# Cardinal-Cryptography/zk-apps

Measured on AMD Instinct MI355X. Metric: shielder_withdraw_groth16_proofs_per_sec_2^20_constraints, higher is better.
Workload: dtype int: signed 28-bit limbs in 32-bit words, 64-bit column accumulators (Fr 255-bit / Fq 381-bit Montgomery); 1 GPU; single withdraw-shaped Groth16 proof, N=2^20 (7 Fr NTTs, 4 G1 MSM + 1 G2 MSM of 2^20-1 terms), 1 proof per step per GPU; relation=update_note (withdraw) with Poseidon-5 hashing, chain-padded to N, curve=BLS12-381, independent_proofs_per_rank=171, distinct_witnesses_per_rank=64, fresh_r_s_per_proof=True, proofs_in_flight_per_gpu=3, msm_schedule=A | B1 (over r*z) + L + H reduced together | B2 (G2)

## Files before the change

### zk-apps_amd/csrc/groth16.hip

```cpp
#include <stdlib.h>
#include <string.h>
#include <new>
#include <string>
#include <memory>
#include <chrono>
#include <functional>
#include <thread>
#include <vector>
#include "ctx.hpp"
#include "tune.hpp"
#include "host_pool.hpp"
#include "pairing.hpp"
#include "r1cs.hpp"
#include "points.hpp"

namespace zkmi {

template <class T>
__device__ __forceinline__ T ldv(const T* p) {
  T r;
  const uint4* s = reinterpret_cast<const uint4*>(p);
  uint4* d = reinterpret_cast<uint4*>(&r);
#pragma unroll
  for (unsigned i = 0; i < sizeof(T) / 16; i++) d[i] = s[i];
  return r;
}
template <class T>
__device__ __forceinline__ void stv(T* p, const T& v) {
  const uint4* s = reinterpret_cast<const uint4*>(&v);
  uint4* d = reinterpret_cast<uint4*>(p);
#pragma unroll
  for (unsigned i = 0; i < sizeof(T) / 16; i++) d[i] = s[i];
}

struct MatSet {
  const uint32_t* rowptr[3];
  const uint32_t* col[3];
  const Fr28* val[3];
};
constexpr uint32_t MATVEC_LONG_ROW = 1024;
__global__ void __launch_bounds__(256)
k_matvec_long(MatSet ms, const uint32_t* __restrict__ rows, const Fr28* __restrict__ z, Fr28* __restrict__ out_base, uint32_t n, uint32_t n_vars) {
  __shared__ Fr28 part[256];
  const uint32_t m = rows[2 * blockIdx.x], i = rows[2 * blockIdx.x + 1];
  const uint32_t* __restrict__ col = ms.col[m];
  const Fr28* __restrict__ val = ms.val[m];
  z += (size_t)blockIdx.y * n_vars;
  Fr28 acc = Fr28::zero();
  const uint32_t b = ms.rowptr[m][i], e = ms.rowptr[m][i + 1];
  for (uint32_t k = b + threadIdx.x; k < e; k += 256) acc = acc + ld28(val + k) * ld28(z + col[k]);
  part[threadIdx.x] = acc;
  __syncthreads();
  for (int o = 128; o > 0; o >>= 1) {
    if ((int)threadIdx.x < o) part[threadIdx.x] = part[threadIdx.x] + part[threadIdx.x + o];
    __syncthreads();
  }
  if (threadIdx.x == 0) st28(out_base + (size_t)m * gridDim.y * n + (size_t)blockIdx.y * n + i, part[0]);
}

template <int S>
__global__ void __launch_bounds__(256)
k_matvec(MatSet ms, const Fr28* __restrict__ z, Fr28* __restrict__ out_base, uint32_t nc, uint32_t n, uint32_t n_pub,
         uint32_t n_vars) {
  const int m = blockIdx.z;
  const uint32_t* __restrict__ rowptr = ms.rowptr[m];
  const uint32_t* __restrict__ col = ms.col[m];
  const Fr28* __restrict__ val = ms.val[m];
  const int is_a = m == 0;
  Fr28* __restrict__ out = out_base + (size_t)m * gridDim.y * n;
  z += (size_t)blockIdx.y * n_vars;
  out += (size_t)blockIdx.y * n;
  const uint32_t gi = blockIdx.x * blockDim.x + threadIdx.x;
  const uint32_t i = gi / S, lane = gi % S;
  if (i >= n) return;
  Fr28 acc = Fr28::zero();
  if (i < nc) {
    const uint32_t b = rowptr[i], e = rowptr[i + 1];
    if (e - b > MATVEC_LONG_ROW) return;
    for (uint32_t k = b + lane; k < e; k += S) acc = acc + ld28(val + k) * ld28(z + col[k]);
  } else if (is_a && i < nc + n_pub && lane == 0) {
    acc = ld28(z + (i - nc));
  }
  if constexpr (S > 1) {
#pragma unroll
    for (int o = S / 2; o > 0; o >>= 1) {
      Fr28 t;
#pragma unroll
      for (int q = 0; q < Fr28::NL; q++) t.l[q] = __shfl_xor(acc.l[q], o);
      acc = acc + t;
    }
    if (lane != 0) return;
  }
  st28(out + i, acc);
}

__global__ void __launch_bounds__(256)
k_check_sat(const Fr28* __restrict__ a, const Fr28* __restrict__ b, const Fr28* __restrict__ c,
            const Fr28* __restrict__ z, uint32_t nc, uint32_t* __restrict__ flag, uint32_t n, uint32_t n_vars) {
  a += (size_t)blockIdx.y * n;
  b += (size_t)blockIdx.y * n;
  c += (size_t)blockIdx.y * n;
  z += (size_t)blockIdx.y * n_vars;
  const uint32_t i = blockIdx.x * blockDim.x + threadIdx.x;
  bool bad = false;
  if (i < nc) {
    const Fr28 d = (ld28(a + i) * ld28(b + i) - ld28(c + i)) * Fr28::one();
    bad = !d.is_zero();
  }
  if (i == 0) {
    const Fr28 d = (ld28(z) - Fr28::one()) * Fr28::one();
    bad = bad || !d.is_zero();
  }
  if (bad) __hip_atomic_fetch_or(flag, 1u, __ATOMIC_RELAXED, __HIP_MEMORY_SCOPE_SYSTEM);
}

__global__ void __launch_bounds__(256)
k_check_canonical(const uint32_t* __restrict__ z, uint32_t n, uint32_t* __restrict__ flag) {
  const uint32_t i = blockIdx.x * blockDim.x + threadIdx.x;
  if (i >= n) return;
  const uint4* q = reinterpret_cast<const uint4*>(z + (size_t)i * 8);
  const uint4 a = q[0], b = q[1];
  const uint32_t w[8] = {a.x, a.y, a.z, a.w, b.x, b.y, b.z, b.w};
  bool lt = false, decided = false;
#pragma unroll
  for (int k = 7; k >= 0; k--)
    if (!decided && w[k] != Fr28Params::MOD32[k]) {
      lt = w[k] < Fr28Params::MOD32[k];
      decided = true;
    }
  if (!lt) __hip_atomic_fetch_or(flag, 2u, __ATOMIC_RELAXED, __HIP_MEMORY_SCOPE_SYSTEM);
}

__global__ void __launch_bounds__(256)
k_quotient(Fr28* __restrict__ a, const Fr28* __restrict__ b, const Fr28* __restrict__ c, Fr28 zinv, uint32_t n) {
  const uint32_t i = blockIdx.x * blockDim.x + threadIdx.x;
  if (i >= n) return;
  st28(a + i, (ld28(a + i) * ld28(b + i) - ld28(c + i)) * zinv);
}

struct ZPtrSet {
  const uint4* p[64];
};
__global__ void __launch_bounds__(64)
k_gather_z(ZPtrSet src, uint4* __restrict__ dst, uint32_t vec16) {
  const uint32_t i = blockIdx.x * 64 + threadIdx.x;
  if (i >= vec16) return;
  dst[(size_t)blockIdx.y * vec16 + i] = src.p[blockIdx.y][i];
}

struct RSet {
  Fr28 r[64];
};
__global__ void __launch_bounds__(64)
k_scale_canonical(const uint32_t* __restrict__ in, RSet rs, uint32_t* __restrict__ out, uint32_t n, uint64_t stride) {
  const uint32_t i = blockIdx.x * 64 + threadIdx.x;
  if (i >= n) return;
  const size_t at = (size_t)blockIdx.y * stride + (size_t)i * 8;
  const uint4* q = reinterpret_cast<const uint4*>(in + at);
  const uint4 a = q[0], b = q[1];
  const uint32_t w[8] = {a.x, a.y, a.z, a.w, b.x, b.y, b.z, b.w};
  const Fr28 v = Fr28::from_canonical(w) * rs.r[blockIdx.y];
  uint32_t o[8];
  v.to_canonical(o);
  uint4* d = reinterpret_cast<uint4*>(out + at);
  d[0] = make_uint4(o[0], o[1], o[2], o[3]);
  d[1] = make_uint4(o[4], o[5], o[6], o[7]);
}

__global__ void __launch_bounds__(64)
k_entries_to_host(const uint32_t* __restrict__ part_total, uint32_t np, uint32_t* __restrict__ host_word) {
  uint32_t s = 0;
  for (uint32_t i = threadIdx.x; i < np; i += 64) s += part_total[i];
  for (int o = 32; o; o >>= 1) s += __shfl_down(s, o, 64);
  if (threadIdx.x == 0) __hip_atomic_store(host_word, s, __ATOMIC_RELAXED, __HIP_MEMORY_SCOPE_SYSTEM);
}

template <class A>
__global__ void __launch_bounds__(256)
k_bitrev_points(const A* __restrict__ in, A* __restrict__ out, int log_n) {
  const uint32_t p = blockIdx.x * blockDim.x + threadIdx.x;
  if (p >= (1u << log_n)) return;
  const uint32_t r = log_n ? (__brev(p) >> (32 - log_n)) : 0u;
  stv(out + p, ldv(in + r));
}

template <class F>
__global__ void __launch_bounds__(64)
k_fixed_base(const uint32_t* __restrict__ scalars, const Affine<F>* __restrict__ table, Affine<F>* __restrict__ out,
             uint32_t n) {
  const uint32_t i = blockIdx.x * blockDim.x + threadIdx.x;
  if (i >= n) return;
  XYZZ<F> acc = XYZZ<F>::infinity();
  for (int w = 0; w < 32; w++) {
    const uint32_t limb = scalars[(size_t)i * 8 + (w >> 2)];
    const uint32_t d = (limb >> ((w & 3) * 8)) & 0xffu;
    if (d) {
      Affine<F> p = ldv(table + w * 256 + d);
      acc.madd(p);
    }
  }
  stv(out + i, acc.to_affine());
}

}

using namespace zkmi;

static bool prover_sort_side() { return ZK_TUNE("ZKMI_SORT_SIDE", 0) == 1; }
static uint32_t prover_solo_max_log() {
  const int v = ZK_TUNE("ZKMI_SOLO_MAX_LOG", 19);
  return (uint32_t)(v < 0 ? 0 : v > 28 ? 28 : v);
}
static bool prover_aux_split() { return ZK_TUNE("ZKMI_AUX_SPLIT", 1) != 0; }

static bool same_bucket_set(const MsmPlan& a, const MsmPlan& b) {
  return a.shared == b.shared && a.c == b.c && a.nwin == b.nwin && a.nb == b.nb && a.seg_log == b.seg_log &&
         a.vec_parts == b.vec_parts && a.ndigits == b.ndigits;
}

struct zkmi_pk {
  zkmi_ctx* ctx = nullptr;
  int device = -1;
  uint32_t n_vars = 0, n_pub = 0, nc = 0, log_n = 0;
  uint32_t tree_height = 0;
  uint32_t gmax = 1;
  uint32_t* d_rowptr[3] = {nullptr, nullptr, nullptr};
  uint32_t* d_long_rows = nullptr;
  uint32_t n_long_rows = 0;
  uint32_t* d_col[3] = {nullptr, nullptr, nullptr};
  Fr28* d_val[3] = {nullptr, nullptr, nullptr};
  G1Affine *a_query = nullptr, *b_g1_query = nullptr, *h_query = nullptr, *l_query = nullptr;
  G2Affine* b_g2_query = nullptr;
  Affine<Fq28>*a28 = nullptr, *b1_28 = nullptr, *h28 = nullptr, *h28_rev = nullptr, *l28 = nullptr;
  Affine<Fq2_28>* b2_28 = nullptr;
  bool shared = false;
  Affine<Fq28>*a_tab = nullptr, *b1_tab = nullptr, *l_tab = nullptr, *h_tab = nullptr;
  Affine<Fq2_28>* b2_tab = nullptr;
  G1Affine alpha_g1, beta_g1, delta_g1, a0, b1_0;
  G2Affine beta_g2, delta_g2, b2_0;
  std::unique_ptr<FixedBase8<Fq>> delta1_tab, k1_tab;
  std::unique_ptr<FixedBase8<Fq2>> delta2_tab;
  G1Affine ka;
  G2Affine kb2;
  Fr* d_z[zkmi_ctx::PROOF_RING] = {};
  mutable const Fr* z_cur[zkmi_ctx::PROOF_RING] = {};
  uint32_t* d_rz[zkmi_ctx::PROOF_RING] = {};
  uint32_t* d_h[zkmi_ctx::PROOF_RING] = {};
  Fr28 *d_zm = nullptr, *d_a = nullptr;
  uint32_t* h_unsat = nullptr;
  uint32_t* h_zent = nullptr;
  mutable bool fold_dense = true;
  mutable uint64_t last_entries = 0, last_full = 0;
  ~zkmi_pk() {
    if (device >= 0) (void)hipSetDevice(device);
    (void)hipDeviceSynchronize();
    for (int m = 0; m < 3; m++) {
      if (d_rowptr[m]) (void)hipFree(d_rowptr[m]);
      if (d_col[m]) (void)hipFree(d_col[m]);
      if (d_val[m]) (void)hipFree(d_val[m]);
    }
    if (d_long_rows) (void)hipFree(d_long_rows);
    void* ptrs[] = {a_query, b_g1_query, h_query, l_query, b_g2_query, d_zm, d_a, a28, b1_28, h28, h28_rev, l28, b2_28,
                    a_tab, b1_tab, l_tab, h_tab, b2_tab, d_z[0], d_z[1], d_z[2], d_h[0], d_h[1], d_h[2]};
    static_assert(zkmi_ctx::PROOF_RING == 3, "ring size");
    for (void* p : ptrs)
      if (p) (void)hipFree(p);
    if (h_unsat) (void)hipHostFree(h_unsat);
    for (uint32_t* p : d_rz)
      if (p) (void)hipFree(p);
  }
};

static hipError_t pk_alloc(zkmi_pk* pk, zkmi_ctx* ctx, const zkmi_r1cs* r) {
  pk->ctx = ctx;
  pk->device = ctx->device;
  pk->n_vars = r->n_vars;
  pk->n_pub = r->n_pub;
  pk->nc = r->n_constraints;
  pk->log_n = r->log_n;
  pk->tree_height = r->tree_height;
  const uint64_t N = 1ull << r->log_n;
  hipError_t e;
  {
    std::vector<uint32_t> longs;
    for (uint32_t m = 0; m < 3; m++)
      for (uint32_t i = 0; i + 1 < r->m[m].rowptr.size(); i++)
        if (r->m[m].rowptr[i + 1] - r->m[m].rowptr[i] > MATVEC_LONG_ROW) {
          longs.push_back(m);
          longs.push_back(i);
        }
// ... 384 lines not shown
  }
  pk_build_delta_tables(pk);
  *out_pk = pk;
  return ZKMI_OK;
}

extern "C" {

int32_t zkmi_pk_check(zkmi_ctx* ctx, const zkmi_pk* pk, int32_t checks, uint64_t out_where[2]) {
  if (!ctx || !pk || checks == 0 || !point_args_ok(PT_ENC_RESIDENT, &checks)) return ZKMI_ERR_BAD_ARG;
  ZK_ENTER(ctx);
  if (ctx->device != pk->device) return ZKMI_ERR_BAD_ARG;
  if (out_where) out_where[0] = out_where[1] = UINT64_MAX;
  const bool sub = (checks & ZKMI_CHECK_SUBGROUP) != 0;
  const G1Affine* s1[3] = {&pk->alpha_g1, &pk->beta_g1, &pk->delta_g1};
  const G2Affine* s2[2] = {&pk->beta_g2, &pk->delta_g2};
  for (uint64_t i = 0; i < 5; i++) {
    const bool curve = i < 3 ? g1_on_curve(*s1[i]) : g2_on_curve(*s2[i - 3]);
    const bool ok = curve && (!sub || (i < 3 ? g1_in_subgroup(*s1[i]) : g2_in_subgroup(*s2[i - 3])));
    if (!ok) {
      if (out_where) out_where[0] = 5, out_where[1] = i;
      return ctx->fail(ZKMI_ERR_NON_CANONICAL, "proving key: single element " + std::to_string(i) + " (section 5): " +
                                                   point_status_name(curve ? ZKMI_PT_NOT_IN_SUBGROUP : ZKMI_PT_NOT_ON_CURVE));
    }
  }
  const uint64_t N = 1ull << pk->log_n, nv = pk->n_vars, np = pk->n_pub;
  struct {
    int group;
    const void* src;
    uint64_t cnt;
  } const sec[5] = {{1, pk->a_query, nv}, {1, pk->b_g1_query, nv}, {2, pk->b_g2_query, nv}, {1, pk->h_query, N - 1},
                    {1, pk->l_query + np, nv - np}};
  for (int k = 0; k < 5; k++) {
    if (!sec[k].cnt) continue;
    uint64_t bad = UINT64_MAX;
    uint32_t st = 0;
    const int32_t rc = points_read(ctx, sec[k].group, sec[k].src, sec[k].cnt, PT_ENC_RESIDENT, checks, nullptr, false, nullptr, &bad, &st);
    if (rc != ZKMI_OK) return rc;
    if (bad != UINT64_MAX) {
      if (out_where) out_where[0] = (uint64_t)k, out_where[1] = bad;
      return ctx->fail(ZKMI_ERR_NON_CANONICAL, std::string("proving key: ") + PK_QUERY_NAME[k] + "[" + std::to_string(bad) +
                                                   "] (section " + std::to_string(k) + "): " + point_status_name(st));
    }
  }
  return ZKMI_OK;
}

int32_t zkmi_pk_free(zkmi_pk* pk) {
  if (!pk) return ZKMI_ERR_BAD_ARG;
  delete pk;
  return ZKMI_OK;
}

int32_t zkmi_pk_shape(const zkmi_pk* pk, uint32_t* n_vars, uint32_t* n_pub, uint32_t* log_n) {
  if (!pk) return ZKMI_ERR_BAD_ARG;
  if (n_vars) *n_vars = pk->n_vars;
  if (n_pub) *n_pub = pk->n_pub;
  if (log_n) *log_n = pk->log_n;
  return ZKMI_OK;
}

int32_t zkmi_pk_schedule_state(const zkmi_pk* pk, uint64_t out[3]) {
  if (!pk || !out) return ZKMI_ERR_BAD_ARG;
  out[0] = (pk->d_rz[0] != nullptr && pk->fold_dense) ? 1 : 0;
  out[1] = pk->last_entries;
  out[2] = pk->last_full;
  return ZKMI_OK;
}

int32_t zkmi_ctx_set_group_size(zkmi_ctx* ctx, uint32_t group) {
  if (!ctx || group > 64) return ZKMI_ERR_BAD_ARG;
  ctx->group_override = group;
  return ZKMI_OK;
}

int32_t zkmi_pk_export_g1_elems(const zkmi_pk* pk, uint8_t out_beta_g1[96], uint8_t out_delta_g1[96]) {
  if (!pk || !out_beta_g1 || !out_delta_g1) return ZKMI_ERR_BAD_ARG;
  g1_to_wire(pk->beta_g1, out_beta_g1);
  g1_to_wire(pk->delta_g1, out_delta_g1);
  return ZKMI_OK;
}

int32_t zkmi_pk_export_query(zkmi_ctx* ctx, const zkmi_pk* pk, int32_t which, uint64_t first, uint64_t count,
                             uint8_t* out) {
  ZK_ENTER(ctx);
  if (!ctx || !pk || !out || which < 0 || which > 4) return ZKMI_ERR_BAD_ARG;
  const uint64_t N = 1ull << pk->log_n;
  if (which == 2) {
    if (first + count > pk->n_vars) return ZKMI_ERR_BAD_ARG;
    std::vector<G2Affine> h(count);
    ZK_HIP(ctx, hipMemcpy(h.data(), pk->b_g2_query + first, sizeof(G2Affine) * count, hipMemcpyDeviceToHost));
    for (uint64_t i = 0; i < count; i++) g2_to_wire(h[i], out + 192 * i);
    return ZKMI_OK;
  }
  const G1Affine* src = which == 0 ? pk->a_query : which == 1 ? pk->b_g1_query : which == 3 ? pk->h_query : pk->l_query + pk->n_pub;
  const uint64_t len = which == 3 ? N - 1 : which == 4 ? pk->n_vars - pk->n_pub : pk->n_vars;
  if (first + count > len) return ZKMI_ERR_BAD_ARG;
  std::vector<G1Affine> h(count);
  ZK_HIP(ctx, hipMemcpy(h.data(), src + first, sizeof(G1Affine) * count, hipMemcpyDeviceToHost));
  for (uint64_t i = 0; i < count; i++) g1_to_wire(h[i], out + 96 * i);
  return ZKMI_OK;
}

static int32_t witness_map_dev(zkmi_ctx* ctx, const zkmi_pk* pk, const void* const* src, bool host, uint32_t G,
                               hipStream_t st, int par = 0) {
  const uint32_t N = 1u << pk->log_n, nv = pk->n_vars;
  PhaseTimer* t = ctx->timer();
  pk->z_cur[par] = pk->d_z[par];
  bool aligned = true;
  for (uint32_t b = 0; b < G; b++) aligned = aligned && (reinterpret_cast<uintptr_t>(src[b]) & 15u) == 0;
  if (host) {
    for (uint32_t b = 0; b < G; b++)
      ZK_HIP(ctx, hipMemcpyAsync(pk->d_z[par] + (size_t)b * nv, src[b], 32ull * nv, hipMemcpyHostToDevice, ctx->stream_copy));
  } else if (G == 1 && aligned) {
    pk->z_cur[par] = static_cast<const Fr*>(src[0]);
  } else if (G <= 64 && aligned) {
    ZPtrSet ps;
    for (uint32_t b = 0; b < 64; b++) ps.p[b] = static_cast<const uint4*>(src[b < G ? b : 0]);
    hipLaunchKernelGGL(k_gather_z, dim3((2 * nv + 63) / 64, G), dim3(64), 0, ctx->stream_copy, ps, reinterpret_cast<uint4*>(pk->d_z[par]), 2 * nv);
  } else {
    for (uint32_t b = 0; b < G; b++)
      ZK_HIP(ctx, hipMemcpyAsync(pk->d_z[par] + (size_t)b * nv, src[b], 32ull * nv, hipMemcpyDeviceToDevice, ctx->stream_copy));
  }
  ZK_HIP(ctx, hipEventRecord(ctx->ev_z[par], ctx->stream_copy));
  ZK_HIP(ctx, hipStreamWaitEvent(ctx->stream, ctx->ev_z[par], 0));
  if (st != ctx->stream) ZK_HIP(ctx, hipStreamWaitEvent(st, ctx->ev_z[par], 0));
  if (t) t->begin(PH_WITNESS, st);
  hipLaunchKernelGGL(k_check_canonical, dim3((G * nv + 63) / 64), dim3(64), 0, st,
                     reinterpret_cast<const uint32_t*>(pk->z_cur[par]), G * nv, pk->h_unsat + par);
  ZK_HIP(ctx, ntt_from_canonical(reinterpret_cast<const uint32_t*>(pk->z_cur[par]), pk->d_zm, G * nv, st));
  MatSet ms;
  for (int m = 0; m < 3; m++) {
    ms.rowptr[m] = pk->d_rowptr[m];
    ms.col[m] = pk->d_col[m];
    ms.val[m] = pk->d_val[m];
  }
  if (G == 1 && pk->log_n <= 16)
    hipLaunchKernelGGL(k_matvec<8>, dim3((8 * N + 63) / 64, 1, 3), dim3(64), 0, st, ms, pk->d_zm, pk->d_a, pk->nc, N, pk->n_pub, nv);
  else
    hipLaunchKernelGGL(k_matvec<1>, dim3((N + 63) / 64, G, 3), dim3(64), 0, st, ms, pk->d_zm, pk->d_a, pk->nc, N, pk->n_pub, nv);
  if (pk->n_long_rows) hipLaunchKernelGGL(k_matvec_long, dim3(pk->n_long_rows, G), dim3(256), 0, st, ms, pk->d_long_rows, pk->d_zm, pk->d_a, N, nv);
  Fr28* const d_b = pk->d_a + (size_t)N * G;
  Fr28* const d_c = pk->d_a + 2 * (size_t)N * G;
  hipLaunchKernelGGL(k_check_sat, dim3((pk->nc + 64) / 64, G), dim3(64), 0, st, pk->d_a, d_b, d_c, pk->d_zm, pk->nc,
                     pk->h_unsat + par, N, nv);
  if (t) t->end(PH_WITNESS, st);
  hipError_t e;
  NttDomain* dom = ctx->domain((int)pk->log_n, &e);
  if (!dom) return ctx->hip_fail(e, "ntt domain");
  if (t) t->begin(PH_NTT, st);
  const bool batch_abc = ZK_TUNE("ZKMI_WITNESS_BATCH", 1) != 0;
  if (batch_abc) {
    ZK_HIP(ctx, dom->inverse_to_rev(pk->d_a, dom->rev_coset_n, nullptr, st, 3 * G));
    ZK_HIP(ctx, dom->forward_from_rev(pk->d_a, st, 3 * G));
  } else {
    for (int m = 0; m < 3; m++) {
      ZK_HIP(ctx, dom->inverse_to_rev(pk->d_a + (size_t)m * N * G, dom->rev_coset_n, nullptr, st, G));
      ZK_HIP(ctx, dom->forward_from_rev(pk->d_a + (size_t)m * N * G, st, G));
    }
  }
  Fr gn = fr_from_u64(7);
  for (uint32_t i = 0; i < pk->log_n; i++) gn = gn.sqr();
  const Fr zinv = (gn - Fr::one()).inv().from_mont();
  const Fr28 zinv28 = Fr28::from_canonical(zinv.l);
  hipLaunchKernelGGL(k_quotient, dim3((G * N + 63) / 64), dim3(64), 0, st, pk->d_a, d_b, d_c, zinv28, G * N);
  ZK_HIP(ctx, dom->inverse_to_rev(pk->d_a, dom->rev_coset_inv_n, pk->d_h[par], st, G));
  if (t) t->end(PH_NTT, st);
  if (st != ctx->stream) ZK_HIP(ctx, hipEventRecord(ctx->ev_h[par], st));
  ZK_HIP(ctx, hipGetLastError());
  return ZKMI_OK;
}

int32_t zkmi_groth16_witness_map(zkmi_ctx* ctx, const zkmi_pk* pk, const uint8_t* z, uint8_t* out_h) {
  ZK_ENTER(ctx);
  if (!ctx || !pk || !z || !out_h) return ZKMI_ERR_BAD_ARG;
  const void* src[1] = {z};
  int32_t rc = witness_map_dev(ctx, pk, src, true, 1, ctx->stream);
  if (rc != ZKMI_OK) return rc;
  const uint32_t N = 1u << pk->log_n;
  std::vector<uint8_t> rev(32ull * N);
  ZK_HIP(ctx, hipMemcpyAsync(rev.data(), pk->d_h[0], 32ull * N, hipMemcpyDeviceToHost, ctx->stream));
  ZK_HIP(ctx, hipStreamSynchronize(ctx->stream));
  const uint32_t flags0 = pk->h_unsat[0];
  pk->h_unsat[0] = 0;
  if (flags0 & 2u) return ctx->fail(ZKMI_ERR_NON_CANONICAL, "witness element >= r");
  for (uint32_t p = 0; p < N; p++) {
    uint32_t i = 0;
    for (uint32_t b = 0; b < pk->log_n; b++) i |= ((p >> b) & 1u) << (pk->log_n - 1 - b);
    memcpy(out_h + 32ull * i, rev.data() + 32ull * p, 32);
  }
  return ZKMI_OK;
}

static int32_t prove_enqueue_z(zkmi_ctx* ctx, const zkmi_pk* pk, const void* const* src, bool host, uint32_t G, int par, bool solo = false,
                               bool followed = false, const uint8_t* r_bytes = nullptr) {
  const uint32_t nv = pk->n_vars;
  hipStream_t st = ctx->stream;
  int32_t rc = witness_map_dev(ctx, pk, src, host, G, ctx->stream_front, par);
  if (rc != ZKMI_OK) return rc;
  PhaseTimer* t = ctx->timer();
  const int s0 = 4 * par, g2s = par;
  const bool heavy_side = ZK_TUNE("ZKMI_HEAVY_ON", 2) == 1;
  if (heavy_side) ZK_HIP(ctx, ctx->lazy_stream(&ctx->stream_heavy, false));
  const hipStream_t sth = heavy_side ? ctx->stream_heavy : nullptr;
  const uint32_t* zs = reinterpret_cast<const uint32_t*>(pk->z_cur[par] + 1);
  const bool sh = pk->shared;
  const bool sort_side = prover_sort_side();
  MsmSort& sz = (sort_side && (ctx->z_flip++ & 1u)) ? ctx->sort_z2 : ctx->sort;
  const bool aux_split = prover_aux_split();
  const hipStream_t ra = ctx->stream_aux, rb = aux_split ? ctx->stream_aux2 : ctx->stream_aux,
                    rc2 = aux_split ? ctx->stream_aux3 : ctx->stream_aux;
  if (sort_side) ZK_HIP(ctx, ctx->lazy_stream(&ctx->stream_sort, true));
  const hipStream_t ss = sort_side ? ctx->stream_sort : st;
  if (sort_side) ZK_HIP(ctx, hipStreamWaitEvent(ss, ctx->ev_z[par], 0));
  if (G > 1)
    ZK_HIP(ctx, sz.run_shared_batch(zs, nv - 1, 8ull * nv, G, ss, t));
  else if (sh)
    ZK_HIP(ctx, sz.run_shared(zs, nv - 1, ss, t));
  else
    ZK_HIP(ctx, sz.run(zs, nv - 1, ss, t));
  if (sh && pk->d_rz[par]) hipLaunchKernelGGL(k_entries_to_host, dim3(1), dim3(64), 0, ss, sz.part_total, (uint32_t)sz.plan.nwin, pk->h_zent + par);
  ZK_HIP(ctx, hipEventRecord(ctx->ev_sort[par], ss));
  if (sort_side) ZK_HIP(ctx, hipStreamWaitEvent(st, ctx->ev_sort[par], 0));
  ZK_HIP(ctx, hipStreamWaitEvent(ctx->stream_g2, ctx->ev_sort[par], 0));
  const bool spread_on = ZK_TUNE("ZKMI_SPREAD", 1) != 0;
  const bool spread = spread_on && G == 1 && pk->log_n <= (solo ? prover_solo_max_log() : 16u) && !sort_side && sh;
  const bool three_streams = spread && !solo;
  if (three_streams) ZK_HIP(ctx, ctx->lazy_stream(&ctx->stream_acc3, false));
  const hipStream_t sb1 = three_streams ? ctx->stream_copy : st, sl = three_streams ? ctx->stream_acc3 : st;
  if (three_streams) {
    ZK_HIP(ctx, hipStreamWaitEvent(sb1, ctx->ev_sort[par], 0));
    ZK_HIP(ctx, hipStreamWaitEvent(sl, ctx->ev_sort[par], 0));
  }
  if (spread && solo) {
    ZK_HIP(ctx, ctx->sort_h.run_shared(pk->d_h[par], 1u << pk->log_n, ctx->stream_front, t));
    ZK_HIP(ctx, hipEventRecord(ctx->ev_sorth[par], ctx->stream_front));
    const bool g2_early = ZK_TUNE("ZKMI_SOLO_G2_EARLY", 1) != 0;
    if (!g2_early) ZK_HIP(ctx, hipStreamWaitEvent(ctx->stream_g2, ctx->ev_sorth[par], 0));
    ZK_HIP(ctx, hipStreamWaitEvent(st, ctx->ev_sorth[par], 0));
    ZK_HIP(ctx, ctx->g2.run_device(sz, pk->b2_tab, ctx->stream_g2, rc2, t, PH_MSM_ACCUM_G2, PH_MSM_REDUCE_G2, g2s, sth));
    const MsmPlan &pz = sz.plan, &ph = ctx->sort_h.plan;
    const bool fuse_h = ZK_TUNE("ZKMI_SOLO_FUSE_H", 1) != 0;
    const bool fused = fuse_h && same_bucket_set(pz, ph);
    ctx->h_mode[par] = fused ? zkmi_ctx::H_FUSED : zkmi_ctx::H_SORTED;
    const MsmSort* sorts[4] = {&sz, &sz, &sz, &ctx->sort_h};
    const Affine<Fq28>* tabs[4] = {pk->a_tab, pk->b1_tab, pk->l_tab, pk->h_tab};
    const hipStream_t reds[4] = {ra, rb, ctx->stream_front, ctx->stream_copy};
    const int slots4[4] = {s0 + 0, s0 + 1, s0 + 2, s0 + 3};
    ZK_HIP(ctx, ctx->g1.run_device_multi(sorts, tabs, fused ? 4 : 3, st, reds, t, PH_MSM_ACCUM_G1, PH_MSM_REDUCE_G1, slots4, sth));
    return ZKMI_OK;
  }
  const int lh_mode = ZK_TUNE("ZKMI_LH_MERGE", 2);
  const uint32_t N = 1u << pk->log_n;
  const bool same_set = sh && same_bucket_set(sz.plan, G > 1 ? msm_make_plan_shared_batch(N, G) : msm_make_plan_shared(N));
  const bool nocall_g1 = ZK_TUNE("ZKMI_ACCUM", 3) == 2 || ZK_TUNE("ZKMI_ACCUM", 3) == 3;
  const bool lh_merge = same_set && ((lh_mode == 2 && !solo) ||
                                     (lh_mode == 1 && nocall_g1 && followed && (G == 1 || ZK_TUNE("ZKMI_LH_MERGE_GROUPS", 0) == 1)));
  const bool fold_b1 = lh_merge && lh_mode == 2 && r_bytes && pk->d_rz[par] != nullptr && (pk->fold_dense || ZK_TUNE("ZKMI_RB1_FOLD_ALWAYS", 0) == 1);
  ctx->h_mode[par] = fold_b1 ? zkmi_ctx::H_INTO_LB : lh_merge ? zkmi_ctx::H_INTO_L : zkmi_ctx::H_OWN;
  if (fold_b1) {
    RSet rs;
    for (uint32_t g = 0; g < G; g++) {
      uint32_t rw[8];
      memcpy(rw, r_bytes + 32ull * g, 32);
      rs.r[g] = Fr28::from_canonical(rw);
    }
    const bool own = ZK_TUNE("ZKMI_RB1_STREAM", 0) == 1;
    if (own) {
      ZK_HIP(ctx, ctx->lazy_stream(&ctx->stream_rz, false));
      ZK_HIP(ctx, hipStreamWaitEvent(ctx->stream_rz, ctx->ev_z[par], 0));
    }
    const hipStream_t sc = own ? ctx->stream_rz : ctx->stream_copy;
    hipLaunchKernelGGL(k_scale_canonical, dim3((nv - 1 + 63) / 64, G), dim3(64), 0, sc, zs, rs, pk->d_rz[par], nv - 1, 8ull * nv);
    if (G > 1)
      ZK_HIP(ctx, ctx->sort_rz.run_shared_batch(pk->d_rz[par], nv - 1, 8ull * nv, G, sc, t));
    else
      ZK_HIP(ctx, ctx->sort_rz.run_shared(pk->d_rz[par], nv - 1, sc, t));
    ZK_HIP(ctx, hipEventRecord(ctx->ev_rz[par], sc));
  }
  ZK_HIP(ctx, ctx->g2.run_device(sz, sh ? pk->b2_tab : pk->b2_28 + 1, ctx->stream_g2, rc2, t,
                                 PH_MSM_ACCUM_G2, PH_MSM_REDUCE_G2, g2s, sth));
  ZK_HIP(ctx, ctx->g1.run_device(sz, sh ? pk->a_tab : pk->a28 + 1, st, ra, t, PH_MSM_ACCUM_G1,
                                 PH_MSM_REDUCE_G1, s0 + 0, sth));
  if (fold_b1) {
    ZK_HIP(ctx, hipStreamWaitEvent(sb1, ctx->ev_rz[par], 0));
    ZK_HIP(ctx, ctx->g1.run_device(ctx->sort_rz, pk->b1_tab, sb1, rb, t, PH_MSM_ACCUM_G1, PH_MSM_REDUCE_G1, s0 + 1, sth, -1, MSM_RUN_NO_REDUCE));
  } else {
    ZK_HIP(ctx, ctx->g1.run_device(sz, sh ? pk->b1_tab : pk->b1_28 + 1, sb1, lh_merge ? ra : rb, t, PH_MSM_ACCUM_G1,
                                   PH_MSM_REDUCE_G1, s0 + 1, sth));
  }
  ZK_HIP(ctx, ctx->g1.run_device(sz, sh ? pk->l_tab : pk->l28 + 1, sl, lh_merge ? rb : ra, t, PH_MSM_ACCUM_G1,
                                 PH_MSM_REDUCE_G1, s0 + 2, sth, -1, lh_merge ? MSM_RUN_NO_REDUCE : 0));
  return ZKMI_OK;
}

static int32_t prove_enqueue_h(zkmi_ctx* ctx, const zkmi_pk* pk, uint32_t G, int par, bool solo = false) {
  const uint32_t N = 1u << pk->log_n;
  (void)solo;
  const int mode = ctx->h_mode[par];
  if (mode == zkmi_ctx::H_FUSED) return ZKMI_OK;
  const bool spread = mode == zkmi_ctx::H_SORTED;
  hipStream_t st = spread ? ctx->stream_copy : ctx->stream;
  if (spread) ZK_HIP(ctx, hipStreamWaitEvent(st, ctx->ev_sorth[par], 0));
  PhaseTimer* t = ctx->timer();
  const bool sh = pk->shared;
  const bool heavy_side = ZK_TUNE("ZKMI_HEAVY_ON", 2) == 1;
  if (heavy_side) ZK_HIP(ctx, ctx->lazy_stream(&ctx->stream_heavy, false));
  const hipStream_t sth = heavy_side ? ctx->stream_heavy : nullptr;
  const bool sort_side = prover_sort_side();
  if (sort_side) ZK_HIP(ctx, ctx->lazy_stream(&ctx->stream_sort, true));
  const hipStream_t ss = sort_side ? ctx->stream_sort : st;
  ZK_HIP(ctx, hipStreamWaitEvent(ss, ctx->ev_h[par], 0));
  if (spread)
    ;
  else if (G > 1)
    ZK_HIP(ctx, ctx->sort_h.run_shared_batch(pk->d_h[par], N, 8ull * N, G, ss, t));
  else if (sh)
    ZK_HIP(ctx, ctx->sort_h.run_shared(pk->d_h[par], N, ss, t));
  else
// ... 503 lines not shown
```

### zk-apps_amd/csrc/msm.hpp

```cpp
#pragma once
#include <hip/hip_runtime.h>
#include <stdint.h>
#include <vector>
#include "curve.hpp"
#include "field28.hpp"
#include "tune.hpp"

namespace zkmi {

struct PhaseTimer {
  enum { MAX_PENDING = 4096 };
  hipEvent_t ev0[MAX_PENDING], ev1[MAX_PENDING];
  int phase_of[MAX_PENDING];
  int n_pending = 0, n_created = 0;
  bool enabled = false;
  double total_ms[16] = {0};
  uint64_t count[16] = {0};
  ~PhaseTimer();
  void begin(int phase, hipStream_t st);
  void end(int phase, hipStream_t st);
  void collect();
  void reset();
};

enum Phase {
  PH_MSM_SORT = 0,
  PH_MSM_ACCUM_G1 = 1,
  PH_MSM_REDUCE_G1 = 2,
  PH_MSM_ACCUM_G2 = 3,
  PH_MSM_REDUCE_G2 = 4,
  PH_NTT = 5,
  PH_WITNESS = 6,
  PH_MISC = 7,
  PH_COUNT = 8
};

constexpr uint64_t MSM_MAX_TERMS = (1ull << 28) - 1;

constexpr int MSM_BIG_WINDOW = 20;
constexpr int MSM_MAX_WINDOW = 22;

struct MsmPlan {
  int c = 0;
  int nwin = 0;
  uint32_t nb = 0;
  uint64_t n = 0;
  bool shared = false;
  int ndigits = 0;
  uint32_t heavy_thr = 256;
  int heavy_shift = 0;
  int seg_log = 4;
  int vec_parts = 1;
  int top_spread_log = 0;
  int win_first = 0, nwin_total = 0;
  int total_windows() const { return nwin_total ? nwin_total : nwin; }
};
MsmPlan msm_make_plan(uint64_t n);
MsmPlan msm_make_plan_c(uint64_t n, int c);
MsmPlan msm_make_plan_shared(uint64_t n);
MsmPlan msm_make_plan_shared_batch(uint64_t n, uint32_t batch);

struct MsmSort {
  uint32_t* count = nullptr;
  uint32_t* begin = nullptr;
  uint32_t* blockhist = nullptr;
  uint32_t* perm = nullptr;
  uint32_t* heavy = nullptr;
  uint32_t* order_bins = nullptr;
  uint32_t* part_total = nullptr;
  uint32_t* blkcnt = nullptr;
  uint32_t* fpart = nullptr;
  uint32_t* rec_entry = nullptr;
  uint32_t* rec_bkt = nullptr;
  uint32_t* rec_aux = nullptr;
  uint32_t* big_ws = nullptr;
  uint32_t* sorted = nullptr;
  uint64_t cap_entries = 0, cap_buckets = 0, cap_hist = 0;
  MsmPlan plan;
  int plan_override = 0;
  int win_first = 0, win_count = 0;
  int big_nb_log = 15;
  mutable std::vector<hipEvent_t> readers;
  hipError_t wait_readers(hipStream_t st);
  ~MsmSort() { release(); }
  void release();
  bool has_shared = false;
  hipError_t reserve(uint64_t n, bool shared_too = false);
  hipError_t allocate(uint64_t ne, uint64_t nbk, uint64_t nh, bool shared);
  hipError_t run(const uint32_t* d_scalars, uint64_t n, hipStream_t st, PhaseTimer* prof);
  hipError_t run_windowed_big(const uint32_t* d_scalars, uint64_t n, hipStream_t st, PhaseTimer* prof);
  hipError_t run_shared(const uint32_t* d_scalars, uint64_t n, hipStream_t st, PhaseTimer* prof);
  hipError_t run_shared_batch(const uint32_t* d_scalars, uint64_t n, uint64_t stride_words, uint32_t batch, hipStream_t st,
                              PhaseTimer* prof);
  hipError_t reserve_batch(uint64_t n, uint32_t batch);
};

hipError_t msm_sort_enable_big_lds();

template <class F> struct HostFieldOf;
template <> struct HostFieldOf<Fq28> { using type = Fq; };
template <> struct HostFieldOf<Fq2_28> { using type = Fq2; };
template <> struct HostFieldOf<BnFq28> { using type = BnFq; };

enum { MSM_RUN_NO_REDUCE = 1, MSM_RUN_ADD_AT_REDUCE = 2, MSM_RUN_TWO_WAVES = 4 };

template <class F>
struct MsmEngine {
  using HF = typename HostFieldOf<F>::type;
  enum { SLOTS = 12, SLOT_PTS = 64 * 32 };
  int nslots = SLOTS;
  XYZZ<F>* buckets = nullptr;
  XYZZ<F>* segsum = nullptr;
  XYZZ<F>* segw = nullptr;
  uint64_t seg_cap = 0;
  XYZZ<F>* heavy_partial = nullptr;
  uint32_t* heavy_ticket = nullptr;
  uint32_t* heavy_plan = nullptr;
  XYZZ<HF>* partial = nullptr;
  XYZZ<F>* tree_stage = nullptr;
  XYZZ<HF>* h_partial = nullptr;
  hipEvent_t done[SLOTS] = {};
  hipEvent_t acc_done[SLOTS] = {};
  hipEvent_t pre[SLOTS] = {};
  hipEvent_t heavy_done[SLOTS] = {};
  hipEvent_t redo_done[SLOTS] = {};
  uint32_t* redo = nullptr;
  MsmPlan slot_plan[SLOTS];
  bool host_spin = true;
  uint64_t cap_buckets = 0;
  uint64_t min_buckets = 0;
  ~MsmEngine() {
    release();
    destroy_events();
  }
  void release();
  hipError_t reset_transients();
  void destroy_events();
  bool has_shared = false;
  hipError_t reserve(uint64_t n, bool shared_too = false);
  hipError_t reserve_buckets(uint64_t buckets);
  hipError_t ensure_slots(int n);
  hipError_t run_device(const MsmSort& sort, const Affine<F>* d_bases, hipStream_t st, hipStream_t st_reduce,
                        PhaseTimer* prof, int ph_accum, int ph_reduce, int slot = 0, hipStream_t st_heavy = nullptr,
                        int bucket_slot = -1, int flags = 0, int bucket_slot3 = -1);
  hipError_t run_device_multi(const MsmSort* const* sorts, const Affine<F>* const* d_bases, int nm, hipStream_t st,
                              const hipStream_t* st_reduces, PhaseTimer* prof, int ph_accum, int ph_reduce, const int* slots,
                              hipStream_t st_heavy = nullptr, const int* bucket_slots = nullptr, int flags = 0, int third_slot = -1);
  hipError_t finish_host(XYZZ<HF>* out, int slot = 0);
  hipError_t finish_host_windows(XYZZ<HF>* out_windows, int slot = 0);
  static void windows_from_partials(const MsmPlan& pl, const XYZZ<HF>* h, XYZZ<HF>* out_windows, bool parallel = false);
  static int partials_per_msm(const MsmPlan& pl);
  hipError_t finish_host_batch(XYZZ<HF>* out, int slot = 0);
  hipError_t wait_slot(int slot);
  XYZZ<HF> host_result_vec(int slot, int v) const;
};

template <class F>
hipError_t bases_convert(const Affine<typename HostFieldOf<F>::type>* d_in, Affine<F>* d_out, uint64_t n, hipStream_t st);

template <class HF>
XYZZ<HF> msm_combine_windows(const XYZZ<HF>* windows, int nwin, int c);

template <class F>
hipError_t msm_build_table(const Affine<F>* d_bases, uint64_t n, const MsmPlan& plan, Affine<F>** out_table,
                           hipStream_t st);

extern template struct MsmEngine<Fq28>;
extern template struct MsmEngine<Fq2_28>;
extern template struct MsmEngine<BnFq28>;
extern template hipError_t msm_build_table<Fq28>(const Affine<Fq28>*, uint64_t, const MsmPlan&, Affine<Fq28>**, hipStream_t);
extern template hipError_t msm_build_table<Fq2_28>(const Affine<Fq2_28>*, uint64_t, const MsmPlan&, Affine<Fq2_28>**, hipStream_t);
extern template hipError_t msm_build_table<BnFq28>(const Affine<BnFq28>*, uint64_t, const MsmPlan&, Affine<BnFq28>**, hipStream_t);
extern template hipError_t bases_convert<Fq28>(const Affine<Fq>*, Affine<Fq28>*, uint64_t, hipStream_t);
extern template hipError_t bases_convert<Fq2_28>(const Affine<Fq2>*, Affine<Fq2_28>*, uint64_t, hipStream_t);
extern template hipError_t bases_convert<BnFq28>(const Affine<BnFq>*, Affine<BnFq28>*, uint64_t, hipStream_t);

}
```

### zk-apps_amd/csrc/msm_impl.hpp

```cpp
#pragma once
#include <stdlib.h>
#include <functional>
#include <type_traits>
#include <vector>
#include "curve.hpp"
#include "host_pool.hpp"
#include "msm.hpp"

namespace zkmi {

static inline uint64_t msm_max_segments(uint64_t buckets) { return (buckets / 16 > (1u << 16) ? buckets / 16 : (1u << 16)) + 1; }
constexpr int MSM_TREE_T = 128;
constexpr uint32_t MSM_STAGE_PTS = 16384;
constexpr uint32_t MSM_STAGE_PTS_1 = 4096;
constexpr uint32_t MSM_HEAVY = 256;

template <class T>
__device__ __forceinline__ T load_vec(const T* p) {
  static_assert(sizeof(T) % 16 == 0, "16-byte multiple");
  T r;
  const uint4* s = reinterpret_cast<const uint4*>(p);
  uint4* d = reinterpret_cast<uint4*>(&r);
#pragma unroll
  for (unsigned i = 0; i < sizeof(T) / 16; i++) d[i] = s[i];
  return r;
}
template <class T>
__device__ __forceinline__ void store_vec(T* p, const T& v) {
  static_assert(sizeof(T) % 16 == 0, "16-byte multiple");
  const uint4* s = reinterpret_cast<const uint4*>(&v);
  uint4* d = reinterpret_cast<uint4*>(p);
#pragma unroll
  for (unsigned i = 0; i < sizeof(T) / 16; i++) d[i] = s[i];
}

typedef __attribute__((address_space(3))) void* lds_ptr_t;
typedef const __attribute__((address_space(1))) void* glb_ptr_t;


__device__ __forceinline__ Fq28 ld_comp(const Fq28* p) {
  Fq28 r;
  const uint2* q = reinterpret_cast<const uint2*>(p);
#pragma unroll
  for (int i = 0; i < 7; i++) {
    const uint2 w = q[i];
    r.l[2 * i] = (int32_t)w.x;
    r.l[2 * i + 1] = (int32_t)w.y;
  }
  return r;
}
__device__ __forceinline__ void st_comp(Fq28* p, const Fq28& v) {
  uint2* q = reinterpret_cast<uint2*>(p);
#pragma unroll
  for (int i = 0; i < 7; i++) q[i] = make_uint2((uint32_t)v.l[2 * i], (uint32_t)v.l[2 * i + 1]);
}


template <class F>
__device__ __forceinline__ bool madd_generic(XYZZ<F>& acc, const Affine<F>& p, uint32_t negmask = 0) {
  F pp_ = f_sub_lazy(p.x * acc.zz, acc.x);
  F r = f_signed_sub_lazy(p.y * acc.zzz, negmask, acc.y);
  F pp = pp_.sqr();
  F rr = r.sqr();
  if (pp.is_zero()) return false;
  F ppp = pp_ * pp;
  acc.zz = acc.zz * pp;
  acc.zzz = acc.zzz * ppp;
  F q = acc.x * pp;
  acc.x = f_x3(rr, ppp, q);
  acc.y = f_mul_sub_mul(r, f_sub_lazy(q, acc.x), acc.y, ppp);
  return true;
}
template <class F>
__device__ __forceinline__ bool madd_affine_pair(XYZZ<F>& acc, const Affine<F>& p, uint32_t negmask = 0) {
  F pp_ = f_sub_lazy(p.x, acc.x);
  F r = f_signed_sub_lazy(p.y, negmask, acc.y);
  F pp = pp_.sqr();
  F rr = r.sqr();
  if (pp.is_zero()) return false;
  F ppp = pp_ * pp;
  F q = acc.x * pp;
  acc.x = f_x3(rr, ppp, q);
  acc.y = f_mul_sub_mul(r, f_sub_lazy(q, acc.x), acc.y, ppp);
  acc.zz = pp;
  acc.zzz = ppp;
  return true;
}
template <class P>
__device__ __forceinline__ bool affine_is_zero_words(const Affine<Fp28<P>>& p) {
  if (p.y.l[0] != 0) return false;
  uint32_t o = 0;
#pragma unroll
  for (int i = 0; i < P::NL; i++) o |= (uint32_t)p.x.l[i] | (uint32_t)p.y.l[i];
  return o == 0;
}

constexpr int MSM_MULTI_MAX = 4;
struct SortView {
  const uint32_t *begin, *count, *perm, *sorted;
  uint32_t heavy_thr;
};
template <class F, bool MULTI>
struct AccumArgs;
template <class F>
struct AccumArgs<F, false> {
  const Affine<F>* bases_;
  XYZZ<F>* buckets_;
  uint32_t* redo_;
  SortView sort_;
  __device__ __forceinline__ const Affine<F>* bases() const { return bases_; }
  __device__ __forceinline__ XYZZ<F>* buckets() const { return buckets_; }
  __device__ __forceinline__ uint32_t* redo() const { return redo_; }
  __device__ __forceinline__ const SortView& sort() const { return sort_; }
};
template <class F>
struct AccumArgs<F, true> {
  const Affine<F>* bases_[MSM_MULTI_MAX];
  XYZZ<F>* buckets_[MSM_MULTI_MAX];
  uint32_t* redo_[MSM_MULTI_MAX];
  SortView sort_[MSM_MULTI_MAX];
  __device__ __forceinline__ const Affine<F>* bases() const { return bases_[blockIdx.y]; }
  __device__ __forceinline__ XYZZ<F>* buckets() const { return buckets_[blockIdx.y]; }
  __device__ __forceinline__ uint32_t* redo() const { return redo_[blockIdx.y]; }
  __device__ __forceinline__ const SortView& sort() const { return sort_[blockIdx.y]; }
};
template <class F, int W, int BW, bool MULTI = false, bool INTO = false>
__global__ void __launch_bounds__(64 * BW, W)
k_accum_g1_nc(const AccumArgs<F, MULTI> args, uint32_t total_buckets) {
  const Affine<F>* __restrict__ const bases = args.bases();
  XYZZ<F>* __restrict__ const buckets = args.buckets();
  uint32_t* __restrict__ const redo = args.redo();
  const uint32_t* __restrict__ const begin = args.sort().begin;
  const uint32_t* __restrict__ const count = args.sort().count;
  const uint32_t* __restrict__ const perm = args.sort().perm;
  const uint32_t* __restrict__ const sorted = args.sort().sorted;
  const uint32_t heavy_thr = args.sort().heavy_thr;
  constexpr int CHUNKS = sizeof(Affine<F>) / 16;
  __shared__ uint4 tile[BW][CHUNKS][64];
  const uint32_t t = blockIdx.x * blockDim.x + threadIdx.x;
  const uint32_t wave = threadIdx.x >> 6, lane = threadIdx.x & 63;
  if (t >= total_buckets) return;
  const uint32_t b = perm[t];
  const uint32_t cnt = count[b];
  if (cnt > heavy_thr) return;
  const uint32_t beg = begin[b], end = beg + cnt;
  auto fetch = [&](uint32_t v) {
    const char* src = reinterpret_cast<const char*>(bases + (v & 0x7fffffffu));
#pragma unroll
    for (int q = 0; q < CHUNKS; q++)
      __builtin_amdgcn_global_load_lds((glb_ptr_t)(src + 16 * q), (lds_ptr_t)&tile[wave][q][0], 16, 0, 0);
  };
  auto take = [&](Affine<F>& p) {
    uint4* d = reinterpret_cast<uint4*>(&p);
#pragma unroll
    for (int q = 0; q < CHUNKS; q++) d[q] = tile[wave][q][lane];
    asm volatile("s_waitcnt lgkmcnt(0)" ::: "memory");
  };
  XYZZ<F> acc;
  uint32_t j = beg;
  for (;; j++) {
    if (j >= end) {
      if constexpr (!INTO) store_vec(buckets + b, XYZZ<F>::infinity());
      return;
    }
// ... 672 lines not shown
        if (sv >> 31) p.y = p.y.neg();
        v.madd(p);
      }
    }
    return v;
  };
  const uint32_t n_heavy = pmode ? hplan[2] : (heavy[0] < h_limit ? heavy[0] : h_limit);
  auto put = [&](uint32_t b, XYZZ<F> v) {
    if (into) v.add(load_vec(buckets + b));
    store_vec(buckets + b, v);
  };
  const uint32_t n_wg = gridDim.x * gridDim.y, wg = blockIdx.y * gridDim.x + blockIdx.x;
  uint32_t item0 = 0;
  const bool tail = h_first >= MSM_HEAVY_CAP;
  for (uint32_t h = tail ? h_first + wg : h_first; h < n_heavy; h += tail ? n_wg : 1u) {
    const uint32_t b = pmode ? ent[4 * h] : heavy[1 + h];
    const uint32_t cnt = pmode ? (ent[4 * (h + 1) + 3] - ent[4 * h + 3]) * 64u : count[b];
    const uint32_t beg0 = pmode ? ent[4 * h + 3] * 64u : begin[b];
    const uint32_t nsplit = tail ? 1u : heavy_nsplit(h, cnt, 4 * MSM_TREE_T, item0);
    const uint32_t base = item0;
    const uint32_t r0 = tail ? 0u : (wg + n_wg - base % n_wg) % n_wg;
    item0 += nsplit;
    for (uint32_t r = r0; r < nsplit; r += n_wg) {
      uint32_t beg = beg0, end = beg0 + cnt;
      if (nsplit > 1) {
        const uint32_t len = (cnt + nsplit - 1) / nsplit;
        const uint32_t sb = beg + r * len;
        end = (sb + len < end) ? sb + len : end;
        beg = sb < end ? sb : end;
      }
      XYZZ<F> acc = XYZZ<F>::infinity();
      if (pmode) {
        for (uint32_t j = beg + threadIdx.x; j < end; j += blockDim.x) acc.add(partial_at(h, j));
      } else {
        for (uint32_t j = beg + threadIdx.x; j < end; j += blockDim.x) {
          const uint32_t v = sorted[j];
          Affine<F> p = load_vec(bases + (v & 0x7fffffffu));
          if (v >> 31) p.y = p.y.neg();
          acc.madd(p);
        }
      }
      acc = block_tree_sum(acc, sh);
      if (nsplit == 1) {
        if (threadIdx.x == 0) put(b, acc);
      } else {
        if (threadIdx.x == 0) {
          store_vec(heavy_partial + (size_t)base + r, acc);
          __threadfence();
          is_last = atomicAdd(ticket + h, 1u) == nsplit - 1 ? 1u : 0u;
        }
        __syncthreads();
        if (is_last) {
          __threadfence();
          XYZZ<F> v = XYZZ<F>::infinity();
          for (uint32_t k = threadIdx.x; k < nsplit; k += blockDim.x) v.add(load_vec(heavy_partial + (size_t)base + k));
          v = block_tree_sum(v, sh);
          if (threadIdx.x == 0) {
            put(b, v);
            ticket[h] = 0;
          }
        }
      }
      __syncthreads();
    }
  }
}

template <class F>
__global__ void __launch_bounds__(256)
k_segreduce(const XYZZ<F>* __restrict__ buckets, XYZZ<F>* __restrict__ segsum, XYZZ<F>* __restrict__ segw,
            uint32_t total_segs, int seg, const XYZZ<F>* __restrict__ buckets2, const XYZZ<F>* __restrict__ buckets3) {
  const uint32_t t = blockIdx.x * blockDim.x + threadIdx.x;
  if (t >= total_segs) return;
  XYZZ<F> run = XYZZ<F>::infinity();
  XYZZ<F> acc = XYZZ<F>::infinity();
  for (int i = seg - 1; i >= 0; i--) {
    XYZZ<F> bk = load_vec(buckets + (size_t)t * seg + i);
    run.add(bk);
    if (buckets2) {
      bk = load_vec(buckets2 + (size_t)t * seg + i);
      run.add(bk);
    }
    if (buckets3) {
      bk = load_vec(buckets3 + (size_t)t * seg + i);
      run.add(bk);
    }
    acc.add(run);
  }
  store_vec(segsum + t, run);
  store_vec(segw + t, acc);
}

template <class F>
__global__ void __launch_bounds__(256, 2)
k_segreduce_w2(const XYZZ<F>* __restrict__ buckets, XYZZ<F>* __restrict__ segsum, XYZZ<F>* __restrict__ segw,
            uint32_t total_segs, int seg, const XYZZ<F>* __restrict__ buckets2, const XYZZ<F>* __restrict__ buckets3) {
  const uint32_t t = blockIdx.x * blockDim.x + threadIdx.x;
  if (t >= total_segs) return;
  XYZZ<F> run = XYZZ<F>::infinity();
  XYZZ<F> acc = XYZZ<F>::infinity();
  for (int i = seg - 1; i >= 0; i--) {
    XYZZ<F> bk = load_vec(buckets + (size_t)t * seg + i);
    run.add(bk);
    if (buckets2) {
      bk = load_vec(buckets2 + (size_t)t * seg + i);
      run.add(bk);
    }
    if (buckets3) {
      bk = load_vec(buckets3 + (size_t)t * seg + i);
      run.add(bk);
    }
    acc.add(run);
  }
  store_vec(segsum + t, run);
  store_vec(segw + t, acc);
}

__device__ __forceinline__ XYZZ<Fq2P> ld_xyzz_split(const XYZZ<Fq2_28>* p, uint32_t comp) {
  const Fq28* s = reinterpret_cast<const Fq28*>(p);
  XYZZ<Fq2P> r;
  r.x.v = ld_comp(s + comp);
  r.y.v = ld_comp(s + 2 + comp);
  r.zz.v = ld_comp(s + 4 + comp);
  r.zzz.v = ld_comp(s + 6 + comp);
  return r;
}
__device__ __forceinline__ void st_xyzz_split(XYZZ<Fq2_28>* p, const XYZZ<Fq2P>& v, uint32_t comp) {
  Fq28* d = reinterpret_cast<Fq28*>(p);
  st_comp(d + comp, v.x.v);
  st_comp(d + 2 + comp, v.y.v);
  st_comp(d + 4 + comp, v.zz.v);
  st_comp(d + 6 + comp, v.zzz.v);
}

template <int UNUSED = 0>
__global__ void __launch_bounds__(256, 2)
k_segreduce_g2_split(const XYZZ<Fq2_28>* __restrict__ buckets, XYZZ<Fq2_28>* __restrict__ segsum,
                     XYZZ<Fq2_28>* __restrict__ segw, uint32_t total_segs, int seg) {
  const uint32_t gt = blockIdx.x * blockDim.x + threadIdx.x;
  const uint32_t t = gt >> 1, comp = gt & 1u;
  if (t >= total_segs) return;
  XYZZ<Fq2P> run = XYZZ<Fq2P>::infinity();
  XYZZ<Fq2P> acc = XYZZ<Fq2P>::infinity();
  for (int i = seg - 1; i >= 0; i--) {
    XYZZ<Fq2P> bk = ld_xyzz_split(buckets + (size_t)t * seg + i, comp);
    run.add(bk);
    acc.add(run);
  }
  st_xyzz_split(segsum + t, run, comp);
  st_xyzz_split(segw + t, acc, comp);
}

template <class F>
__global__ void __launch_bounds__(MSM_TREE_T)
k_treesum(const XYZZ<F>* __restrict__ segsum, const XYZZ<F>* __restrict__ segw, uint32_t segs_per_win,
          XYZZ<typename HostFieldOf<F>::type>* __restrict__ partial, int plain_job, XYZZ<F>* __restrict__ stage,
          XYZZ<typename HostFieldOf<F>::type>* __restrict__ partial_host) {
  extern __shared__ __align__(16) unsigned char lds_raw[];
  XYZZ<F>* sh = reinterpret_cast<XYZZ<F>*>(lds_raw);
  const int job = blockIdx.x;
  const int w = blockIdx.y;
  const uint32_t nchunk = gridDim.z, z = blockIdx.z;
  const XYZZ<F>* src = (job == 0 ? segw : segsum) + (size_t)w * segs_per_win;
  const bool whole = job == 0 || job == plain_job;
  const uint32_t len = whole ? segs_per_win : segs_per_win / 2;
  const uint32_t per = (len + nchunk - 1) / nchunk;
  const uint32_t lo = z * per, hi = lo + per < len ? lo + per : len;
  XYZZ<F> acc = XYZZ<F>::infinity();
  if (whole) {
    for (uint32_t t = lo + threadIdx.x; t < hi; t += blockDim.x) {
      XYZZ<F> v = load_vec(src + t);
      acc.add(v);
    }
  } else {
    const uint32_t b = (uint32_t)(job - 1), lowmask = (1u << b) - 1u;
    for (uint32_t u = lo + threadIdx.x; u < hi; u += blockDim.x) {
      const uint32_t t = ((u & ~lowmask) << 1) | (1u << b) | (u & lowmask);
      XYZZ<F> v = load_vec(src + t);
      acc.add(v);
    }
  }
  sh[threadIdx.x] = acc;
  __syncthreads();
  for (uint32_t s = blockDim.x / 2; s > 0; s >>= 1) {
    if (threadIdx.x < s) {
      acc.add(sh[threadIdx.x + s]);
      sh[threadIdx.x] = acc;
    }
    __syncthreads();
  }
  if (threadIdx.x == 0) {
    if (nchunk == 1) {
      XYZZ<typename HostFieldOf<F>::type> o = {fq_from_fq28(acc.x), fq_from_fq28(acc.y), fq_from_fq28(acc.zz),
                                               fq_from_fq28(acc.zzz)};
      store_vec(partial + (size_t)w * gridDim.x + job, o);
      store_vec(partial_host + (size_t)w * gridDim.x + job, o);
    } else {
      store_vec(stage + ((size_t)w * gridDim.x + job) * nchunk + z, acc);
    }
  }
}

template <class F>
__global__ void __launch_bounds__(MSM_TREE_T)
k_treesum_final(const XYZZ<F>* __restrict__ stage, uint32_t nchunk, XYZZ<typename HostFieldOf<F>::type>* __restrict__ partial,
                XYZZ<typename HostFieldOf<F>::type>* __restrict__ partial_host) {
  extern __shared__ __align__(16) unsigned char lds_raw[];
  XYZZ<F>* sh = reinterpret_cast<XYZZ<F>*>(lds_raw);
  const size_t idx = (size_t)blockIdx.y * gridDim.x + blockIdx.x;
  XYZZ<F> acc = XYZZ<F>::infinity();
  if (threadIdx.x < nchunk) acc = load_vec(stage + idx * nchunk + threadIdx.x);
  sh[threadIdx.x] = acc;
  __syncthreads();
  for (uint32_t s = blockDim.x / 2; s > 0; s >>= 1) {
    if (threadIdx.x < s) {
      acc.add(sh[threadIdx.x + s]);
      sh[threadIdx.x] = acc;
    }
    __syncthreads();
  }
  if (threadIdx.x == 0) {
    XYZZ<typename HostFieldOf<F>::type> o = {fq_from_fq28(acc.x), fq_from_fq28(acc.y), fq_from_fq28(acc.zz),
                                             fq_from_fq28(acc.zzz)};
    store_vec(partial + idx, o);
    store_vec(partial_host + idx, o);
  }
}

__device__ __forceinline__ void st_host_split(XYZZ<Fq2>* dst, const XYZZ<Fq2P>& v, uint32_t comp) {
  Fq* d = reinterpret_cast<Fq*>(dst);
  d[comp] = fq_from_fq28(v.x.v);
  d[2 + comp] = fq_from_fq28(v.y.v);
  d[4 + comp] = fq_from_fq28(v.zz.v);
  d[6 + comp] = fq_from_fq28(v.zzz.v);
}
__device__ __forceinline__ XYZZ<Fq2P> pair_tree_sum(XYZZ<Fq2P> acc, XYZZ<Fq2_28>* sh, uint32_t pair, uint32_t npair, uint32_t comp) {
  st_xyzz_split(sh + pair, acc, comp);
  __syncthreads();
  for (uint32_t s = npair / 2; s > 0; s >>= 1) {
    if (pair < s) {
      XYZZ<Fq2P> o = ld_xyzz_split(sh + pair + s, comp);
      acc.add(o);
      st_xyzz_split(sh + pair, acc, comp);
    }
    __syncthreads();
  }
  return acc;
}
template <int UNUSED = 0>
__global__ void __launch_bounds__(2 * MSM_TREE_T, 2)
k_treesum_g2_split(const XYZZ<Fq2_28>* __restrict__ segsum, const XYZZ<Fq2_28>* __restrict__ segw, uint32_t segs_per_win,
                   XYZZ<Fq2>* __restrict__ partial, int plain_job, XYZZ<Fq2_28>* __restrict__ stage, XYZZ<Fq2>* __restrict__ partial_host) {
  extern __shared__ __align__(16) unsigned char lds_raw[];
  XYZZ<Fq2_28>* sh = reinterpret_cast<XYZZ<Fq2_28>*>(lds_raw);
  const int job = blockIdx.x;
  const int w = blockIdx.y;
  const uint32_t nchunk = gridDim.z, z = blockIdx.z;
  const uint32_t pair = threadIdx.x >> 1, comp = threadIdx.x & 1u, npair = blockDim.x >> 1;
  const XYZZ<Fq2_28>* src = (job == 0 ? segw : segsum) + (size_t)w * segs_per_win;
  const bool whole = job == 0 || job == plain_job;
  const uint32_t len = whole ? segs_per_win : segs_per_win / 2;
  const uint32_t per = (len + nchunk - 1) / nchunk;
  const uint32_t lo = z * per, hi = lo + per < len ? lo + per : len;
  const uint32_t b = whole ? 0u : (uint32_t)(job - 1), lowmask = (1u << b) - 1u;
  XYZZ<Fq2P> acc = XYZZ<Fq2P>::infinity();
  for (uint32_t u = lo + pair; u < hi; u += npair) {
    const uint32_t t = whole ? u : (((u & ~lowmask) << 1) | (1u << b) | (u & lowmask));
    XYZZ<Fq2P> v = ld_xyzz_split(src + t, comp);
    acc.add(v);
  }
  acc = pair_tree_sum(acc, sh, pair, npair, comp);
  if (pair == 0) {
    if (nchunk == 1)
    {
      st_host_split(partial + (size_t)w * gridDim.x + job, acc, comp);
      st_host_split(partial_host + (size_t)w * gridDim.x + job, acc, comp);
    }
    else
      st_xyzz_split(stage + ((size_t)w * gridDim.x + job) * nchunk + z, acc, comp);
  }
}
template <int UNUSED = 0>
__global__ void __launch_bounds__(2 * MSM_TREE_T, 2)
k_treesum_final_g2_split(const XYZZ<Fq2_28>* __restrict__ stage, uint32_t nchunk, XYZZ<Fq2>* __restrict__ partial,
                         XYZZ<Fq2>* __restrict__ partial_host) {
  extern __shared__ __align__(16) unsigned char lds_raw[];
  XYZZ<Fq2_28>* sh = reinterpret_cast<XYZZ<Fq2_28>*>(lds_raw);
  const size_t idx = (size_t)blockIdx.y * gridDim.x + blockIdx.x;
  const uint32_t pair = threadIdx.x >> 1, comp = threadIdx.x & 1u, npair = blockDim.x >> 1;
  XYZZ<Fq2P> acc = XYZZ<Fq2P>::infinity();
  if (pair < nchunk) acc = ld_xyzz_split(stage + idx * nchunk + pair, comp);
  acc = pair_tree_sum(acc, sh, pair, npair, comp);
  if (pair == 0) {
    st_host_split(partial + idx, acc, comp);
    st_host_split(partial_host + idx, acc, comp);
  }
}

__device__ __forceinline__ Affine<Fq2P> ld_affine_split(const Affine<Fq2_28>* bases, uint32_t v, uint32_t comp) {
  const Fq28* src = reinterpret_cast<const Fq28*>(bases + (v & 0x7fffffffu));
  Affine<Fq2P> p;
  p.x.v = ld_comp(src + comp);
  p.y.v = ld_comp(src + 2 + comp);
  if (v >> 31) p.y = p.y.neg();
  return p;
}
template <int UNUSED = 0>
__global__ void __launch_bounds__(MSM_TREE_T, 2)
k_accum_heavy_g2_split(const Affine<Fq2_28>* __restrict__ bases, const uint32_t* __restrict__ begin,
                       const uint32_t* __restrict__ count, const uint32_t* __restrict__ heavy,
                       const uint32_t* __restrict__ sorted, XYZZ<Fq2_28>* __restrict__ buckets,
                       XYZZ<Fq2_28>* __restrict__ heavy_partial, uint32_t* __restrict__ ticket, uint32_t h_first,
                       uint32_t h_limit, const uint32_t* __restrict__ hplan, const XYZZ<Fq2_28>* __restrict__ pool_nc) {
  extern __shared__ __align__(16) unsigned char lds_raw[];
  XYZZ<Fq2_28>* sh = reinterpret_cast<XYZZ<Fq2_28>*>(lds_raw);
  __shared__ uint32_t is_last;
  const uint32_t pair = threadIdx.x >> 1, comp = threadIdx.x & 1u, npair = blockDim.x >> 1;
  const bool pmode = hplan != nullptr && hplan[3] == 0;
  const uint32_t* __restrict__ const ent = hplan + 4;
  const uint32_t pl_nc = pmode ? hplan[1] : 0u;
  auto partial_at = [&](uint32_t h, uint32_t j) {
    XYZZ<Fq2P> v = ld_xyzz_split(pool_nc + j, comp);
    uint32_t o = 0;
#pragma unroll
    for (int i = 0; i < Fq28::NL; i++) o |= (uint32_t)v.zz.v.l[i];
    uint32_t mk = (comp == 0 && v.zzz.v.l[0] == 1) ? 1u : 0u;
    o |= (uint32_t)__builtin_amdgcn_mov_dpp((int)o, 0xB1, 0xF, 0xF, true);
    mk |= (uint32_t)__builtin_amdgcn_mov_dpp((int)mk, 0xB1, 0xF, 0xF, true);
    if (o == 0 && mk == 1) {
      const uint32_t it = j >> 5, pr = j & 31u;
      const uint32_t beg = ent[4 * h + 1], cnt = ent[4 * h + 2], first = ent[4 * h + 3];
      const uint32_t w0 = beg + (it - first) * 32u * pl_nc;
      const uint32_t w1 = (w0 + 32u * pl_nc < beg + cnt) ? w0 + 32u * pl_nc : beg + cnt;
      v = XYZZ<Fq2P>::infinity();
      for (uint32_t jj = w0 + pr; jj < w1; jj += 32) v.madd(ld_affine_split(bases, sorted[jj], comp));
    } else if (o == 0) {
      v = XYZZ<Fq2P>::infinity();
    }
    return v;
  };
  const uint32_t n_heavy = pmode ? hplan[2] : (heavy[0] < h_limit ? heavy[0] : h_limit);
  const uint32_t n_wg = gridDim.x * gridDim.y, wg = blockIdx.y * gridDim.x + blockIdx.x;
  uint32_t item0 = 0;
  const bool tail = h_first >= MSM_HEAVY_CAP;
  for (uint32_t h = tail ? h_first + wg : h_first; h < n_heavy; h += tail ? n_wg : 1u) {
    const uint32_t b = pmode ? ent[4 * h] : heavy[1 + h];
    const uint32_t cnt = pmode ? (ent[4 * (h + 1) + 3] - ent[4 * h + 3]) * 32u : count[b];
    const uint32_t beg0 = pmode ? ent[4 * h + 3] * 32u : begin[b];
    const uint32_t nsplit = tail ? 1u : heavy_nsplit(h, cnt, 4 * npair, item0);
    const uint32_t base = item0;
    const uint32_t r0 = tail ? 0u : (wg + n_wg - base % n_wg) % n_wg;
    item0 += nsplit;
    for (uint32_t r = r0; r < nsplit; r += n_wg) {
      uint32_t beg = beg0, end = beg0 + cnt;
      if (nsplit > 1) {
        const uint32_t len = (cnt + nsplit - 1) / nsplit;
        const uint32_t sb = beg + r * len;
        end = (sb + len < end) ? sb + len : end;
        beg = sb < end ? sb : end;
      }
      XYZZ<Fq2P> acc = XYZZ<Fq2P>::infinity();
      if (pmode) {
        for (uint32_t j = beg + pair; j < end; j += npair) acc.add(partial_at(h, j));
      } else {
        for (uint32_t j = beg + pair; j < end; j += npair) acc.madd(ld_affine_split(bases, sorted[j], comp));
      }
      acc = pair_tree_sum(acc, sh, pair, npair, comp);
      if (nsplit == 1) {
        if (pair == 0) st_xyzz_split(buckets + b, acc, comp);
      } else {
        if (pair == 0) {
          st_xyzz_split(heavy_partial + (size_t)base + r, acc, comp);
          __threadfence();
        }
        __syncthreads();
        if (threadIdx.x == 0) is_last = atomicAdd(ticket + h, 1u) == nsplit - 1 ? 1u : 0u;
        __syncthreads();
        if (is_last) {
          __threadfence();
          XYZZ<Fq2P> v = XYZZ<Fq2P>::infinity();
          for (uint32_t k = pair; k < nsplit; k += npair) v.add(ld_xyzz_split(heavy_partial + (size_t)base + k, comp));
          v = pair_tree_sum(v, sh, pair, npair, comp);
          if (pair == 0) st_xyzz_split(buckets + b, v, comp);
          if (threadIdx.x == 0) ticket[h] = 0;
        }
      }
      __syncthreads();
    }
  }
}
template <int UNUSED = 0>
__global__ void __launch_bounds__(64, 2)
k_accum_redo_g2_split(const Affine<Fq2_28>* __restrict__ bases, const uint32_t* __restrict__ begin,
                      const uint32_t* __restrict__ count, const uint32_t* __restrict__ sorted,
                      XYZZ<Fq2_28>* __restrict__ buckets, uint32_t* __restrict__ redo, uint32_t* __restrict__ ticket) {
  extern __shared__ __align__(16) unsigned char lds_raw[];
  XYZZ<Fq2_28>* sh = reinterpret_cast<XYZZ<Fq2_28>*>(lds_raw);
  const uint32_t n = redo[0];
  const uint32_t pair = threadIdx.x >> 1, comp = threadIdx.x & 1u, npair = blockDim.x >> 1;
  for (uint32_t k = blockIdx.x; k < n; k += gridDim.x) {
    const uint32_t b = redo[1 + k];
    const uint32_t beg = begin[b], end = beg + count[b];
    XYZZ<Fq2P> acc = XYZZ<Fq2P>::infinity();
    for (uint32_t j = beg + pair; j < end; j += npair) acc.madd(ld_affine_split(bases, sorted[j], comp));
    acc = pair_tree_sum(acc, sh, pair, npair, comp);
    if (pair == 0) st_xyzz_split(buckets + b, acc, comp);
    __syncthreads();
  }
  __syncthreads();
  if (threadIdx.x == 0 && atomicAdd(ticket, 1u) == gridDim.x - 1) {
    redo[0] = 0;
    *ticket = 0;
  }
}

}
#include "msm_quad.hpp"
namespace zkmi {

template <class F>
__global__ void __launch_bounds__(256)
k_bases_convert(const Affine<typename HostFieldOf<F>::type>* __restrict__ in, Affine<F>* __restrict__ out,
                uint32_t n) {
  uint32_t i = blockIdx.x * blockDim.x + threadIdx.x;
  if (i >= n) return;
  Affine<typename HostFieldOf<F>::type> p = load_vec(in + i);
  Affine<F> q = {fq28_from_fq(p.x), fq28_from_fq(p.y)};
  store_vec(out + i, q);
}

template <class F>
void MsmEngine<F>::release() {
  if (buckets) (void)hipFree(buckets);
  if (segsum) (void)hipFree(segsum);
  if (segw) (void)hipFree(segw);
  if (partial) (void)hipFree(partial);
  if (tree_stage) (void)hipFree(tree_stage);
  tree_stage = nullptr;
  if (heavy_partial) (void)hipFree(heavy_partial);
  heavy_partial = nullptr;
  if (heavy_plan) (void)hipFree(heavy_plan);
  heavy_plan = nullptr;
  if (heavy_ticket) (void)hipFree(heavy_ticket);
  heavy_ticket = nullptr;
  if (redo) (void)hipFree(redo);
  redo = nullptr;
  if (h_partial) (void)hipHostFree(h_partial);
  buckets = segsum = segw = nullptr;
  partial = h_partial = nullptr;
  cap_buckets = 0;
}

uint64_t msm_max_buckets(uint64_t n);

template <class F>
hipError_t MsmEngine<F>::reset_transients() {
  if (!redo || !heavy_ticket) return hipSuccess;
  hipError_t e = hipMemset(redo, 0, sizeof(uint32_t) * (cap_buckets + 2) * nslots);
  if (e != hipSuccess) return e;
  return hipMemset(heavy_ticket, 0, sizeof(uint32_t) * MSM_HEAVY_CAP * nslots);
}

template <class F>
void MsmEngine<F>::destroy_events() {
  for (int i = 0; i < SLOTS; i++) {
    hipEvent_t* evs[] = {&done[i], &acc_done[i], &pre[i], &heavy_done[i], &redo_done[i]};
    for (hipEvent_t* e : evs) {
      if (*e) (void)hipEventDestroy(*e);
      *e = nullptr;
    }
  }
}

template <class F>
hipError_t MsmEngine<F>::ensure_slots(int n) {
  if (n > SLOTS) return hipErrorInvalidValue;
  if (n <= nslots) return hipSuccess;
  const bool sh = has_shared;
  const uint64_t mb = min_buckets;
  release();
  has_shared = sh;
  min_buckets = mb;
  nslots = n;
  return hipSuccess;
}

template <class F>
hipError_t MsmEngine<F>::reserve_buckets(uint64_t buckets) {
  if (buckets <= cap_buckets) return hipSuccess;
  const bool sh = has_shared;
  release();
  has_shared = sh;
  min_buckets = buckets;
  return reserve(1, sh);
}

template <class F>
hipError_t MsmEngine<F>::reserve(uint64_t n, bool shared_too) {
  uint64_t need = msm_max_buckets(n);
  if (need < min_buckets) need = min_buckets;
  const uint64_t forced = (uint64_t)(255 / 16 + 1) * (1u << 15);
  if (need < forced) need = forced;
  shared_too = shared_too || has_shared;
  if (shared_too) {
    const MsmPlan sp = msm_make_plan_shared(n);
    const uint64_t sb = (uint64_t)sp.nwin * sp.nb;
    if (need < sb) need = sb;
  }
  has_shared = shared_too;
  if (need <= cap_buckets) return hipSuccess;
  release();
  hipError_t e;
  if ((e = hipMalloc(&buckets, sizeof(XYZZ<F>) * need * nslots)) != hipSuccess) return e;
  seg_cap = msm_max_segments(need);
  if ((e = hipMalloc(&segsum, sizeof(XYZZ<F>) * seg_cap * nslots)) != hipSuccess) return e;
  if ((e = hipMalloc(&segw, sizeof(XYZZ<F>) * seg_cap * nslots)) != hipSuccess) return e;
  if ((e = hipMalloc(&partial, sizeof(XYZZ<HF>) * SLOTS * SLOT_PTS)) != hipSuccess) return e;
  if ((e = hipMalloc(&tree_stage, sizeof(XYZZ<F>) * MSM_STAGE_PTS * nslots)) != hipSuccess) return e;
  if ((e = hipMalloc(&heavy_partial, sizeof(XYZZ<F>) * ((size_t)MSM_HPOOL + MSM_HNC_POOL) * nslots)) != hipSuccess) return e;
  if ((e = hipMalloc(&heavy_plan, sizeof(uint32_t) * MSM_HPLAN_WORDS * nslots)) != hipSuccess) return e;
  if ((e = hipMalloc(&heavy_ticket, sizeof(uint32_t) * MSM_HEAVY_CAP * nslots)) != hipSuccess) return e;
  if ((e = hipMemset(heavy_ticket, 0, sizeof(uint32_t) * MSM_HEAVY_CAP * nslots)) != hipSuccess) return e;
  if ((e = hipMalloc(&redo, sizeof(uint32_t) * (need + 2) * nslots)) != hipSuccess) return e;
  if ((e = hipMemset(redo, 0, sizeof(uint32_t) * (need + 2) * nslots)) != hipSuccess) return e;
  if ((e = hipHostMalloc(&h_partial, sizeof(XYZZ<HF>) * SLOTS * SLOT_PTS, hipHostMallocCoherent)) != hipSuccess) return e;
  for (int i = 0; i < SLOTS; i++) {
    hipEvent_t* evs[] = {&done[i], &acc_done[i], &pre[i], &heavy_done[i], &redo_done[i]};
    for (hipEvent_t* ev : evs)
      if (!*ev && (e = hipEventCreateWithFlags(ev, hipEventDisableTiming)) != hipSuccess) return e;
  }
  cap_buckets = need;
  return hipSuccess;
}

static inline int msm_seg_bits(const MsmPlan& pl) {
  const uint32_t segs_per_win = pl.nb >> pl.seg_log;
  int seg_bits = 0;
  while ((1u << seg_bits) < segs_per_win) seg_bits++;
  return seg_bits;
}

template <class F>
hipError_t MsmEngine<F>::run_device(const MsmSort& sort, const Affine<F>* d_bases, hipStream_t st,
                                    hipStream_t st_reduce, PhaseTimer* prof, int ph_accum, int ph_reduce, int slot,
                                    hipStream_t st_heavy, int bucket_slot, int flags, int bucket_slot3) {
  const MsmSort* sp = &sort;
  return run_device_multi(&sp, &d_bases, 1, st, &st_reduce, prof, ph_accum, ph_reduce, &slot, st_heavy,
                          bucket_slot >= 0 ? &bucket_slot : nullptr, flags, bucket_slot3);
}

template <class F>
hipError_t MsmEngine<F>::run_device_multi(const MsmSort* const* sorts, const Affine<F>* const* d_bases, int nm, hipStream_t st,
                                          const hipStream_t* st_reduces, PhaseTimer* prof, int ph_accum, int ph_reduce,
                                          const int* slots, hipStream_t st_heavy, const int* bucket_slots, int flags, int third_slot) {
  if (nm < 1 || nm > MSM_MULTI_MAX) return hipErrorInvalidValue;
  if (third_slot >= nslots || (third_slot >= 0 && (nm != 1 || !(flags & MSM_RUN_ADD_AT_REDUCE) || !bucket_slots))) return hipErrorInvalidValue;
  const bool no_reduce = (flags & MSM_RUN_NO_REDUCE) != 0;
  const bool add_at_reduce = (flags & MSM_RUN_ADD_AT_REDUCE) != 0;
  bool any_into = false;
  for (int m = 0; m < nm; m++) {
    if (slots[m] < 0 || slots[m] >= nslots) return hipErrorInvalidValue;
    if (bucket_slots && (bucket_slots[m] < 0 || bucket_slots[m] >= nslots)) return hipErrorInvalidValue;
    any_into = any_into || (!add_at_reduce && bucket_slots && bucket_slots[m] != slots[m]);
  }
  if (add_at_reduce && std::is_same<F, Fq2_28>::value) return hipErrorInvalidValue;
  if (any_into && (nm != 1 || std::is_same<F, Fq2_28>::value)) return hipErrorInvalidValue;
  const MsmPlan& pl = sorts[0]->plan;
  for (int m = 1; m < nm; m++) {
    const MsmPlan& q = sorts[m]->plan;
    if (q.nwin != pl.nwin || q.nb != pl.nb || q.seg_log != pl.seg_log || q.shared != pl.shared || q.c != pl.c) return hipErrorInvalidValue;
  }
  const uint32_t tot_b = pl.nwin * pl.nb;
  const int T = 256;
  hipError_t e;
  const int heavy_on = ZK_TUNE("ZKMI_HEAVY_ON", 2);
  const int accum_mode = ZK_TUNE("ZKMI_ACCUM", 3);
  const int accum_mode_g2 = ZK_TUNE("ZKMI_ACCUM_G2", 2);
  const int mode = std::is_same<F, Fq2_28>::value ? accum_mode_g2 : accum_mode;
  const bool nocall = mode == 2 || mode == 3;
  constexpr bool g2_engine = std::is_same<F, Fq2_28>::value;
  const int quad_mask = g2_engine ? (host_spin ? ZK_TUNE("ZKMI_QUAD_G2", 15) : ZK_TUNE("ZKMI_QUAD_G2_BATCH", 12))
                                  : (host_spin ? ZK_TUNE("ZKMI_QUAD", 15) : ZK_TUNE("ZKMI_QUAD_BATCH", 12));
  using QPT = typename std::conditional<g2_engine, XYZZQ<Fq28, 0, true>, XYZZQ<F, 0, false>>::type;
  constexpr uint32_t QPW = g2_engine ? 8u : 16u;
  const bool quad_reduce_ok = pl.shared || pl.c <= 16;
#ifdef ZKMI_EXPERIMENTS
  const int accum_block = ZK_TUNE("ZKMI_ACCUM_BLOCK", 64) == 256 ? 256 : 64;
  const int accum_rounds = ZK_TUNE("ZKMI_ACCUM_ROUNDS", 0);
  auto striped = [&](uint32_t threads_needed, uint32_t block) {
    uint32_t blocks = (threads_needed + block - 1) / block;
    if (accum_rounds > 1) blocks = (blocks + accum_rounds - 1) / accum_rounds;
    return blocks ? blocks : 1u;
  };
#else
  if (!nocall) return hipErrorInvalidValue;
#endif
  if (any_into && !nocall) return hipErrorInvalidValue;
  auto bslot_of = [&](int m) { return bucket_slots ? bucket_slots[m] : slots[m]; };
  auto into_of = [&](int m) { return !add_at_reduce && bslot_of(m) != slots[m]; };
  auto second_of = [&](int m) { return add_at_reduce && bslot_of(m) != slots[m]; };
  auto bk_of = [&](int m) { return buckets + (size_t)(into_of(m) ? bslot_of(m) : slots[m]) * cap_buckets; };
  {
    const uint32_t spw = pl.nb >> pl.seg_log;
    if ((uint64_t)pl.nwin * spw > seg_cap || (uint64_t)(2 + msm_seg_bits(pl)) * pl.nwin > SLOT_PTS || tot_b > cap_buckets)
      return hipErrorInvalidValue;
  }
  auto redo_of = [&](int m) { return this->redo + (size_t)slots[m] * (cap_buckets + 2); };

  bool heavy_first[MSM_MULTI_MAX];
  hipStream_t heavy_stream[MSM_MULTI_MAX];
  const bool heavy_deferred = host_spin && tot_b <= (1u << 16) && (quad_mask & 8) && heavy_on == 2 && ZK_TUNE("ZKMI_HEAVY_DEFER", 0) != 0;
  auto launch_heavy = [&](int m) {
    const MsmSort& sort = *sorts[m];
    XYZZ<F>* const hp = heavy_partial + (size_t)slots[m] * ((size_t)MSM_HPOOL + MSM_HNC_POOL);
    XYZZ<F>* const pool_nc = hp + MSM_HPOOL;
    uint32_t* const hplan = heavy_plan + (size_t)slots[m] * MSM_HPLAN_WORDS;
    uint32_t* const tk = heavy_ticket + (size_t)slots[m] * MSM_HEAVY_CAP;
    const bool wide_tail = !pl.shared && pl.c > 16;
    const bool nc = ZK_TUNE("ZKMI_HEAVY_NC", 1) != 0 && !wide_tail && !into_of(m);
    constexpr uint32_t lanes = std::is_same<F, Fq2_28>::value ? 32u : 64u;
    if (nc) {
      hipLaunchKernelGGL(k_heavy_plan<0>, dim3(1), dim3(64), 0, heavy_stream[m], sort.heavy, sort.count, sort.begin, hplan, lanes, 0u);
      if constexpr (std::is_same<F, Fq2_28>::value)
        hipLaunchKernelGGL((k_accum_heavy_nc_g2<2>), dim3(4096), dim3(64), 0, heavy_stream[m], d_bases[m], sort.sorted, hplan, pool_nc);
      else
        hipLaunchKernelGGL((k_accum_heavy_nc<F, 3>), dim3(6144), dim3(64), 0, heavy_stream[m], d_bases[m], sort.sorted, hplan, pool_nc);
    }
    const uint32_t* const plan_arg = nc ? hplan : nullptr;
    if (nc && (quad_mask & 8)) {
      hipLaunchKernelGGL(k_heavy_q<QPT>, dim3(1024), dim3(64), 0, heavy_stream[m], d_bases[m], sort.begin, sort.count, sort.heavy,
                         sort.sorted, bk_of(m), hp, tk, hplan, pool_nc);
    } else if constexpr (std::is_same<F, Fq2_28>::value) {
      hipLaunchKernelGGL(k_accum_heavy_g2_split<0>, dim3(MSM_HSPLIT, 8), dim3(MSM_TREE_T), sizeof(XYZZ<F>) * MSM_TREE_T / 2, heavy_stream[m],
                         d_bases[m], sort.begin, sort.count, sort.heavy, sort.sorted, bk_of(m), hp, tk, 0u,
                         wide_tail ? MSM_HEAVY_CAP : 0xffffffffu, plan_arg, pool_nc);
      if (wide_tail)
        hipLaunchKernelGGL(k_accum_heavy_g2_split<0>, dim3(1, 4096), dim3(MSM_TREE_T), sizeof(XYZZ<F>) * MSM_TREE_T / 2, heavy_stream[m],
                           d_bases[m], sort.begin, sort.count, sort.heavy, sort.sorted, bk_of(m), hp, tk, MSM_HEAVY_CAP, 0xffffffffu,
                           (const uint32_t*)nullptr, pool_nc);
    } else {
      hipLaunchKernelGGL(k_accum_heavy<F>, dim3(MSM_HSPLIT, 8), dim3(MSM_TREE_T), sizeof(XYZZ<F>) * MSM_TREE_T, heavy_stream[m],
                         d_bases[m], sort.begin, sort.count, sort.heavy, sort.sorted, bk_of(m), hp, tk, into_of(m) ? 1u : 0u, 0u,
                         wide_tail ? MSM_HEAVY_CAP : 0xffffffffu, plan_arg, pool_nc);
      if (wide_tail)
        hipLaunchKernelGGL(k_accum_heavy<F>, dim3(1, 4096), dim3(MSM_TREE_T), sizeof(XYZZ<F>) * MSM_TREE_T, heavy_stream[m],
                           d_bases[m], sort.begin, sort.count, sort.heavy, sort.sorted, bk_of(m), hp, tk, into_of(m) ? 1u : 0u, MSM_HEAVY_CAP,
                           0xffffffffu, (const uint32_t*)nullptr, pool_nc);
    }
  };
#ifdef ZKMI_EXPERIMENTS
  if (const int mask_bits = ZK_TUNE("ZKMI_GATHER_MASK_BITS", 0); mask_bits > 0 && mask_bits < 31)
    for (int m = 0; m < nm; m++)
      hipLaunchKernelGGL(k_mask_sorted<0>, dim3(1024), dim3(256), 0, st, sorts[m]->sorted, sorts[m]->cap_entries,
                         0x80000000u | ((1u << mask_bits) - 1u));
#endif
  for (int m = 0; m < nm; m++) {
    slot_plan[slots[m]] = sorts[m]->plan;
    const hipStream_t st_reduce = st_reduces[m];
    const bool on_reduce = heavy_on == 2 && st_reduce != st;
    const bool side = !on_reduce && heavy_on != 0 && st_heavy && st_heavy != st;
    heavy_first[m] = side || on_reduce;
    heavy_stream[m] = on_reduce ? st_reduce : side ? st_heavy : st;
    if (into_of(m)) {
      if ((e = hipStreamWaitEvent(st, redo_done[bslot_of(m)], 0)) != hipSuccess) return e;
      if (heavy_stream[m] != st && (e = hipStreamWaitEvent(heavy_stream[m], redo_done[bslot_of(m)], 0)) != hipSuccess) return e;
      if (st_reduce != st && st_reduce != heavy_stream[m] && (e = hipStreamWaitEvent(st_reduce, redo_done[bslot_of(m)], 0)) != hipSuccess) return e;
    }
    if (heavy_first[m]) {
      if ((e = hipEventRecord(pre[slots[m]], st)) != hipSuccess) return e;
      if ((e = hipStreamWaitEvent(heavy_stream[m], pre[slots[m]], 0)) != hipSuccess) return e;
      if (!heavy_deferred) launch_heavy(m);
    }
  }
  auto view_of = [&](int m) {
    const MsmSort& sort = *sorts[m];
    return SortView{sort.begin, sort.count, sort.perm, sort.sorted, sort.plan.heavy_thr};
  };

  const bool force_multi = ZK_TUNE("ZKMI_FORCE_MULTI", 0) != 0;
  if (prof) prof->begin(ph_accum, st);
  if constexpr (std::is_same<F, Fq2_28>::value) {
    for (int m = 0; m < nm; m++) {
      const MsmSort& sort = *sorts[m];
      const uint32_t heavy_thr = sort.plan.heavy_thr;
      XYZZ<F>* const bk = bk_of(m);
      uint32_t* const redo = redo_of(m);
#ifdef ZKMI_EXPERIMENTS
      if (mode == 3) {
        hipLaunchKernelGGL((k_accum_g2_nc<3, 1>), dim3((2 * tot_b + 63) / 64), dim3(64), 0, st, d_bases[m], sort.begin, sort.count,
                           sort.perm, sort.sorted, bk, tot_b, heavy_thr, redo);
        continue;
      }
      if (mode != 2) {
        if (accum_block == 64)
          hipLaunchKernelGGL(k_accum_g2_split<1>, dim3(striped(2 * tot_b, 64)), dim3(64), 0, st, d_bases[m], sort.begin, sort.count,
                             sort.perm, sort.sorted, bk, tot_b, heavy_thr);
        else
          hipLaunchKernelGGL(k_accum_g2_split<4>, dim3(striped(2 * tot_b, 256)), dim3(256), 0, st, d_bases[m], sort.begin, sort.count,
                             sort.perm, sort.sorted, bk, tot_b, heavy_thr);
        continue;
      }
#endif
#ifdef ZKMI_EXPERIMENTS
      if ((quad_mask & 16) && tot_b <= (1u << 16)) {
        if constexpr (g2_engine) {
          AccumQArgs<QPT> qa;
          for (int k = 0; k < MSM_MULTI_MAX; k++) {
            qa.bases[k] = d_bases[m];
            qa.buckets[k] = bk;
            qa.sort[k] = view_of(m);
          }
          hipLaunchKernelGGL(k_accum_q<QPT>, dim3((tot_b + QPW - 1) / QPW, 1), dim3(64), 0, st, qa, tot_b);
        }
        continue;
      }
#endif
      if (host_spin && tot_b <= (1u << 15) && ZK_TUNE("ZKMI_SOLO_SPLIT_G2", 1) != 0) {
        hipLaunchKernelGGL(k_accum_g2_split2<0>, dim3((4 * tot_b + 63) / 64), dim3(64), 0, st, d_bases[m], sort.begin, sort.count,
                           sort.perm, sort.sorted, bk, tot_b, heavy_thr, redo);
        continue;
      }
      hipLaunchKernelGGL((k_accum_g2_nc<2, 1>), dim3((2 * tot_b + 63) / 64), dim3(64), 0, st, d_bases[m], sort.begin, sort.count,
                         sort.perm, sort.sorted, bk, tot_b, heavy_thr, redo);
    }
  } else if ((nm > 1 || (force_multi && !any_into)) && nocall) {
    AccumArgs<F, true> set;
    for (int m = 0; m < MSM_MULTI_MAX; m++) {
      const int k = m < nm ? m : 0;
      set.bases_[m] = d_bases[k];
      set.buckets_[m] = bk_of(k);
      set.redo_[m] = redo_of(k);
      set.sort_[m] = view_of(k);
    }
    const bool split2 = ZK_TUNE("ZKMI_SOLO_SPLIT", 1) != 0;
#ifdef ZKMI_EXPERIMENTS
    if ((quad_mask & 16) && tot_b <= (1u << 16)) {
      if constexpr (!g2_engine) {
        AccumQArgs<QPT> qa;
        for (int m = 0; m < MSM_MULTI_MAX; m++) {
          const int k = m < nm ? m : 0;
          qa.bases[m] = d_bases[k];
          qa.buckets[m] = bk_of(k);
          qa.sort[m] = view_of(k);
        }
        hipLaunchKernelGGL(k_accum_q<QPT>, dim3((tot_b + QPW - 1) / QPW, nm), dim3(64), 0, st, qa, tot_b);
      }
    } else
#endif
    if (split2 && tot_b <= (1u << 16))
      hipLaunchKernelGGL((k_accum_g1_split2<F, 1>), dim3((2 * tot_b + 63) / 64, nm), dim3(64), 0, st, set, tot_b);
#ifdef ZKMI_EXPERIMENTS
    else if (accum_mode != 3)
      hipLaunchKernelGGL((k_accum_g1_nc<F, 2, 1, true>), dim3((tot_b + 63) / 64, nm), dim3(64), 0, st, set, tot_b);
#endif
    else
      hipLaunchKernelGGL((k_accum_g1_nc<F, 3, 1, true>), dim3((tot_b + 63) / 64, nm), dim3(64), 0, st, set, tot_b);
  } else {
    for (int m = 0; m < nm; m++) {
      const MsmSort& sort = *sorts[m];
      XYZZ<F>* const bk = bk_of(m);
      uint32_t* const redo = redo_of(m);
      const AccumArgs<F, false> one = {d_bases[m], bk, redo, view_of(m)};
      if (into_of(m)) {
#ifdef ZKMI_EXPERIMENTS
        hipLaunchKernelGGL((k_accum_g1_nc<F, 3, 1, false, true>), dim3((tot_b + 63) / 64), dim3(64), 0, st, one, tot_b);
        continue;
#else
        return hipErrorInvalidValue;
#endif
      }
#ifdef ZKMI_EXPERIMENTS
      if (accum_mode != 3) {
        const uint32_t heavy_thr = sort.plan.heavy_thr;
        const dim3 grid((tot_b + T - 1) / T);
        if (accum_mode == 2)
          hipLaunchKernelGGL((k_accum_g1_nc<F, 2, 1>), dim3((tot_b + 63) / 64), dim3(64), 0, st, one, tot_b);
        else if (accum_mode == 1)
          hipLaunchKernelGGL(k_accum<F>, grid, dim3(T), 0, st, d_bases[m], sort.begin, sort.count, sort.perm, sort.sorted, bk, tot_b,
                             heavy_thr);
        else if (accum_block == 64)
          hipLaunchKernelGGL((k_accum_g1_glds<F, 1>), dim3(striped(tot_b, 64)), dim3(64), 0, st, d_bases[m], sort.begin, sort.count,
                             sort.perm, sort.sorted, bk, tot_b, heavy_thr);
        else
          hipLaunchKernelGGL((k_accum_g1_glds<F, 4>), dim3(striped(tot_b, 256)), dim3(256), 0, st, d_bases[m], sort.begin, sort.count,
                             sort.perm, sort.sorted, bk, tot_b, heavy_thr);
        continue;
      }
#endif
      (void)sort;
#ifdef ZKMI_EXPERIMENTS
      if ((flags & MSM_RUN_TWO_WAVES) || ZK_TUNE("ZKMI_ACCUM_W2", 0) == 1) {
        hipLaunchKernelGGL(k_accum_g1_nc_w2<F>, dim3((tot_b + 63) / 64), dim3(64), 0, st, one, tot_b);
        continue;
      }
#endif
      hipLaunchKernelGGL((k_accum_g1_nc<F, 3, 1>), dim3((tot_b + 63) / 64), dim3(64), 0, st, one, tot_b);
    }
  }
  if (prof) prof->end(ph_accum, st);
  if (heavy_deferred)
    for (int m = 0; m < nm; m++)
      if (heavy_first[m]) launch_heavy(m);

  const uint32_t segs_per_win = pl.nb >> pl.seg_log;
  const uint32_t tot_segs = pl.nwin * segs_per_win;
  const int seg = 1 << pl.seg_log;
  const int plain_job = pl.shared ? 1 + msm_seg_bits(pl) : -1;
  const int njobs = 1 + msm_seg_bits(pl) + (pl.shared ? 1 : 0);
  constexpr bool is_g2 = std::is_same<F, Fq2_28>::value;
  const uint32_t per_block = is_g2 ? MSM_TREE_T : 2 * MSM_TREE_T;
  uint32_t nchunk = 1;
  if (tot_b <= (1u << 16) && segs_per_win > per_block) {
    nchunk = segs_per_win / per_block;
    if (nchunk > MSM_TREE_T) nchunk = MSM_TREE_T;
    if ((uint64_t)njobs * pl.nwin * nchunk > MSM_STAGE_PTS_1) nchunk = 1;
  } else if (!pl.shared && tot_b <= (1u << 19) && segs_per_win > per_block) {
    nchunk = MSM_TREE_T;
    while (nchunk > 1 && ((uint64_t)njobs * pl.nwin * nchunk > 1024 || nchunk * per_block > segs_per_win)) nchunk >>= 1;
  } else if (!pl.shared && pl.c > 16) {
    nchunk = MSM_TREE_T;
    while (nchunk > 1 && ((uint64_t)njobs * pl.nwin * nchunk > MSM_STAGE_PTS_1 || nchunk * per_block > segs_per_win)) nchunk >>= 1;
  }
  for (int m = 0; m < nm; m++) {
    const MsmSort& sort = *sorts[m];
    const int slot = slots[m];
    const hipStream_t st_reduce = st_reduces[m];
    XYZZ<F>* const bk = bk_of(m);
    if (!heavy_first[m]) launch_heavy(m);
    if ((e = hipEventRecord(acc_done[slot], st)) != hipSuccess) return e;
    sort.readers.push_back(acc_done[slot]);
    if (st_reduce != st && (e = hipStreamWaitEvent(st_reduce, acc_done[slot], 0)) != hipSuccess) return e;
    if (heavy_first[m] && heavy_stream[m] != st_reduce) {
      if ((e = hipEventRecord(heavy_done[slot], heavy_stream[m])) != hipSuccess) return e;
      if ((e = hipStreamWaitEvent(st_reduce, heavy_done[slot], 0)) != hipSuccess) return e;
      sort.readers.push_back(heavy_done[slot]);
    }
    if (heavy_first[m] && heavy_stream[m] == st_reduce && !nocall) {
      if ((e = hipEventRecord(heavy_done[slot], st_reduce)) != hipSuccess) return e;
      sort.readers.push_back(heavy_done[slot]);
    }
    if (nocall) {
      uint32_t* const redo = redo_of(m);
      if (quad_mask & 4)
        hipLaunchKernelGGL(k_accum_redo_q<QPT>, dim3(64), dim3(64), 0, st_reduce, d_bases[m], sort.begin, sort.count, sort.sorted, bk, redo,
                           redo + cap_buckets + 1, into_of(m) ? 1u : 0u);
      else if constexpr (std::is_same<F, Fq2_28>::value)
        hipLaunchKernelGGL(k_accum_redo_g2_split<0>, dim3(64), dim3(64), sizeof(XYZZ<F>) * 32, st_reduce, d_bases[m], sort.begin, sort.count, sort.sorted, bk,
                           redo, redo + cap_buckets + 1);
      else
        hipLaunchKernelGGL(k_accum_redo<F>, dim3(64), dim3(64), sizeof(XYZZ<F>) * 64, st_reduce, d_bases[m], sort.begin, sort.count, sort.sorted, bk, redo,
                           redo + cap_buckets + 1, into_of(m) ? 1u : 0u);
      if ((e = hipEventRecord(redo_done[slot], st_reduce)) != hipSuccess) return e;
      sort.readers.push_back(redo_done[slot]);
    }
    if (no_reduce) continue;
    if (prof) prof->begin(ph_reduce, st_reduce);
    XYZZ<F>* const ssum = segsum + (size_t)slot * seg_cap;
    XYZZ<F>* const sw = segw + (size_t)slot * seg_cap;
    if constexpr (is_g2) {
      if ((quad_mask & 1) && quad_reduce_ok)
        hipLaunchKernelGGL(k_segreduce_q<QPT>, dim3((tot_segs + QPW - 1) / QPW), dim3(64), 0, st_reduce, bk, ssum, sw, tot_segs, seg,
                           (const XYZZ<F>*)nullptr, (const XYZZ<F>*)nullptr);
      else
        hipLaunchKernelGGL(k_segreduce_g2_split<0>, dim3((2 * tot_segs + T - 1) / T), dim3(T), 0, st_reduce, bk, ssum, sw,
                           tot_segs, seg);
    } else {
      const XYZZ<F>*bk2 = nullptr, *bk3 = nullptr;
      if (second_of(m)) {
        if ((e = hipStreamWaitEvent(st_reduce, redo_done[bslot_of(m)], 0)) != hipSuccess) return e;
        bk2 = buckets + (size_t)bslot_of(m) * cap_buckets;
        if (third_slot >= 0) {
          if ((e = hipStreamWaitEvent(st_reduce, redo_done[third_slot], 0)) != hipSuccess) return e;
          bk3 = buckets + (size_t)third_slot * cap_buckets;
        }
      }
      if (!pl.shared && pl.c > 16)
        hipLaunchKernelGGL(k_segreduce_w2<F>, dim3((tot_segs + T - 1) / T), dim3(T), 0, st_reduce, bk, ssum, sw, tot_segs, seg, bk2, bk3);
      else if (quad_mask & 1)
        hipLaunchKernelGGL(k_segreduce_q<QPT>, dim3((tot_segs + QPW - 1) / QPW), dim3(64), 0, st_reduce, bk, ssum, sw, tot_segs, seg, bk2, bk3);
      else
        hipLaunchKernelGGL(k_segreduce<F>, dim3((tot_segs + T - 1) / T), dim3(T), 0, st_reduce, bk, ssum, sw, tot_segs, seg, bk2, bk3);
    }
    XYZZ<HF>* dp = partial + (size_t)slot * SLOT_PTS;
    XYZZ<HF>* const hp_out = h_partial + (size_t)slot * SLOT_PTS;
    XYZZ<F>* const stg = tree_stage + (size_t)slot * MSM_STAGE_PTS;
    if ((quad_mask & 2) && quad_reduce_ok) {
      uint32_t nq = 1;
      while ((uint64_t)nq * nq * 4 <= segs_per_win) nq <<= 1;
      while (nq > 1 && ((uint64_t)njobs * pl.nwin * nq > MSM_STAGE_PTS || nq * QPW > segs_per_win)) nq >>= 1;
      hipLaunchKernelGGL(k_treesum_q<QPT>, dim3(njobs, pl.nwin, nq), dim3(64), 0, st_reduce, ssum, sw, segs_per_win, dp, plain_job, stg, hp_out);
      if (nq > 1) hipLaunchKernelGGL(k_treesum_final_q<QPT>, dim3(njobs, pl.nwin), dim3(64), 0, st_reduce, stg, nq, dp, hp_out);
    } else if constexpr (is_g2) {
      if (nchunk > 1) {
        hipLaunchKernelGGL(k_treesum_g2_split<0>, dim3(njobs, pl.nwin, nchunk), dim3(MSM_TREE_T), sizeof(XYZZ<F>) * MSM_TREE_T / 2, st_reduce,
                           ssum, sw, segs_per_win, dp, plain_job, stg, hp_out);
        uint32_t tf = 64;
        while (tf < 2 * nchunk) tf <<= 1;
        hipLaunchKernelGGL(k_treesum_final_g2_split<0>, dim3(njobs, pl.nwin), dim3(tf), sizeof(XYZZ<F>) * tf / 2, st_reduce, stg, nchunk, dp, hp_out);
      } else {
#ifdef ZKMI_EXPERIMENTS
        if (ZK_TUNE("ZKMI_G2_TREE_SPLIT", 1) == 0)
          hipLaunchKernelGGL(k_treesum<F>, dim3(njobs, pl.nwin, 1), dim3(MSM_TREE_T), sizeof(XYZZ<F>) * MSM_TREE_T, st_reduce,
                             ssum, sw, segs_per_win, dp, plain_job, stg, hp_out);
        else
#endif
          hipLaunchKernelGGL(k_treesum_g2_split<0>, dim3(njobs, pl.nwin, 1), dim3(2 * MSM_TREE_T), sizeof(XYZZ<F>) * MSM_TREE_T, st_reduce,
                             ssum, sw, segs_per_win, dp, plain_job, stg, hp_out);
      }
    } else {
      hipLaunchKernelGGL(k_treesum<F>, dim3(njobs, pl.nwin, nchunk), dim3(MSM_TREE_T), sizeof(XYZZ<F>) * MSM_TREE_T, st_reduce,
                         ssum, sw, segs_per_win, dp, plain_job, stg, hp_out);
      if (nchunk > 1) {
        uint32_t tf = 64;
        while (tf < nchunk) tf <<= 1;
        hipLaunchKernelGGL(k_treesum_final<F>, dim3(njobs, pl.nwin), dim3(tf), sizeof(XYZZ<F>) * tf, st_reduce, stg, nchunk, dp, hp_out);
      }
    }
    if (prof) prof->end(ph_reduce, st_reduce);
    if ((e = hipEventRecord(done[slot], st_reduce)) != hipSuccess) return e;
  }
  return hipGetLastError();
}

template <class F>
hipError_t MsmEngine<F>::finish_host_windows(XYZZ<HF>* out_windows, int slot) {
  hipError_t e = wait_event(done[slot], host_spin);
  if (e != hipSuccess) return e;
  windows_from_partials(slot_plan[slot], h_partial + (size_t)slot * SLOT_PTS, out_windows, host_spin);
  return hipSuccess;
}

template <class F>
int MsmEngine<F>::partials_per_msm(const MsmPlan& pl) { return pl.nwin * (1 + msm_seg_bits(pl) + (pl.shared ? 1 : 0)); }
template <class F>
void MsmEngine<F>::windows_from_partials(const MsmPlan& pl, const XYZZ<HF>* h, XYZZ<HF>* out_windows, bool parallel) {
  const int seg_bits = msm_seg_bits(pl);
  const int njobs = 1 + seg_bits + (pl.shared ? 1 : 0);
  const std::function<void(uint32_t)> one = [&](uint32_t w) {
    XYZZ<HF> u = XYZZ<HF>::infinity();
    const int bits = (pl.win_first + (int)w == pl.total_windows() - 1 && pl.top_spread_log > 0) ? seg_bits - pl.top_spread_log : seg_bits;
    for (int j = bits - 1; j >= 0; j--) {
      u.dbl_inplace();
      u.add(h[(size_t)w * njobs + 1 + j]);
    }
    for (int i = 0; i < pl.seg_log; i++) u.dbl_inplace();
    u.add(h[(size_t)w * njobs]);
    out_windows[w] = u;
  };
  if (parallel && pl.nwin >= 8) {
    HostPool::instance().run((uint32_t)pl.nwin, host_cpu_budget(), one);
  } else {
    for (int w = 0; w < pl.nwin; w++) one((uint32_t)w);
  }
}

template <class HF>
static XYZZ<HF> msm_combine_partitions(const XYZZ<HF>* win, const XYZZ<HF>* h, int parts, int njobs, uint32_t nb) {
  XYZZ<HF> run = XYZZ<HF>::infinity(), t = XYZZ<HF>::infinity(), total = XYZZ<HF>::infinity();
  for (int q = parts - 1; q >= 1; q--) {
    run.add(h[(size_t)q * njobs + (njobs - 1)]);
    t.add(run);
  }
  for (uint32_t b = nb; b > 1; b >>= 1) t.dbl_inplace();
  for (int q = 0; q < parts; q++) total.add(win[q]);
  total.add(t);
  return total;
}

template <class F>
hipError_t MsmEngine<F>::finish_host_batch(XYZZ<HF>* out, int slot) {
  const MsmPlan& pl = slot_plan[slot];
  if (pl.vec_parts <= 1) return finish_host_windows(out, slot);
  std::vector<XYZZ<HF>> win(pl.nwin);
  hipError_t e = finish_host_windows(win.data(), slot);
  if (e != hipSuccess) return e;
  const int njobs = 2 + msm_seg_bits(pl);
  const XYZZ<HF>* h = h_partial + (size_t)slot * SLOT_PTS;
  for (int v = 0; v * pl.vec_parts < pl.nwin; v++)
    out[v] = msm_combine_partitions<HF>(win.data() + (size_t)v * pl.vec_parts, h + (size_t)v * pl.vec_parts * njobs, pl.vec_parts,
                                        njobs, pl.nb);
  return hipSuccess;
}

template <class F>
hipError_t MsmEngine<F>::wait_slot(int slot) {
  return wait_event(done[slot], host_spin);
}
template <class F>
XYZZ<typename MsmEngine<F>::HF> MsmEngine<F>::host_result_vec(int slot, int v) const {
  const MsmPlan& pl = slot_plan[slot];
  const int vp = pl.vec_parts > 1 ? pl.vec_parts : 1;
  const int njobs = 1 + msm_seg_bits(pl) + (pl.shared ? 1 : 0);
  const XYZZ<HF>* h = h_partial + (size_t)slot * SLOT_PTS + (size_t)v * vp * njobs;
  MsmPlan mine = pl;
  mine.nwin = vp;
  XYZZ<HF> win[64];
  windows_from_partials(mine, h, win);
  if (vp == 1) return win[0];
  return msm_combine_partitions<HF>(win, h, vp, njobs, pl.nb);
}

template <class HF>
XYZZ<HF> msm_combine_windows(const XYZZ<HF>* windows, int nwin, int c) {
  XYZZ<HF> total = XYZZ<HF>::infinity();
  for (int w = nwin - 1; w >= 0; w--) {
    for (int i = 0; i < c; i++) total.dbl_inplace();
    total.add(windows[w]);
  }
  return total;
}

template <class F>
hipError_t MsmEngine<F>::finish_host(XYZZ<HF>* out, int slot) {
  const MsmPlan& pl = slot_plan[slot];
  std::vector<XYZZ<HF>> win(pl.nwin);
  hipError_t e = finish_host_windows(win.data(), slot);
  if (e != hipSuccess) return e;
  if (!pl.shared) {
    *out = msm_combine_windows(win.data(), pl.nwin, pl.c);
    return hipSuccess;
  }
  *out = msm_combine_partitions<HF>(win.data(), h_partial + (size_t)slot * SLOT_PTS, pl.nwin, 2 + msm_seg_bits(pl), pl.nb);
  return hipSuccess;
}

template <class F>
__global__ void __launch_bounds__(64)
k_build_table(const Affine<F>* __restrict__ bases, Affine<F>* __restrict__ table, uint32_t n, int ndigits, int c) {
  const uint32_t i = blockIdx.x * blockDim.x + threadIdx.x;
  if (i >= n) return;
  const Affine<F> p = load_vec(bases + i);
  XYZZ<F> cur = XYZZ<F>::from_affine(p);
  store_vec(table + i, p);
  for (int w = 1; w < ndigits; w++) {
    for (int k = 0; k < c; k++) cur.dbl_inplace();
    const Affine<F> a = cur.to_affine();
    Affine<F> o = cur.is_inf() ? Affine<F>::infinity() : a;
    store_vec(table + (size_t)w * n + i, o);
  }
}

template <class F>
hipError_t msm_build_table(const Affine<F>* d_bases, uint64_t n, const MsmPlan& plan, Affine<F>** out_table,
                           hipStream_t st) {
  *out_table = nullptr;
  hipError_t e = hipMalloc(out_table, sizeof(Affine<F>) * (size_t)plan.ndigits * (n ? n : 1));
  if (e != hipSuccess) return e;
  if (n) {
    hipLaunchKernelGGL(k_build_table<F>, dim3((unsigned)((n + 63) / 64)), dim3(64), 0, st, d_bases, *out_table,
                       (uint32_t)n, plan.ndigits, plan.c);
    e = hipGetLastError();
  }
  return e;
}

template <class F>
hipError_t bases_convert(const Affine<typename HostFieldOf<F>::type>* d_in, Affine<F>* d_out, uint64_t n,
                         hipStream_t st) {
  if (!n) return hipSuccess;
  hipLaunchKernelGGL(k_bases_convert<F>, dim3((unsigned)((n + 255) / 256)), dim3(256), 0, st, d_in, d_out, (uint32_t)n);
  return hipGetLastError();
}

}
```

### zk-apps_amd/csrc/ntt.hip

```cpp
#include <stdlib.h>
#include <type_traits>
#include <utility>
#include "ntt.hpp"
#include "tune.hpp"

namespace zkmi {

namespace {

__device__ __forceinline__ void ld_words8(const uint32_t* p, uint32_t* w) {
  const uint4* q = reinterpret_cast<const uint4*>(p);
  const uint4 a = q[0], b = q[1];
  w[0] = a.x; w[1] = a.y; w[2] = a.z; w[3] = a.w;
  w[4] = b.x; w[5] = b.y; w[6] = b.z; w[7] = b.w;
}
__device__ __forceinline__ void st_words8(uint32_t* p, const uint32_t* w) {
  uint4* q = reinterpret_cast<uint4*>(p);
  q[0] = make_uint4(w[0], w[1], w[2], w[3]);
  q[1] = make_uint4(w[4], w[5], w[6], w[7]);
}

template <class F>
__global__ void k_bitrev_copy(const F* __restrict__ in, F* __restrict__ out, int log_n) {
  const uint32_t i = blockIdx.x * blockDim.x + threadIdx.x;
  if (i >= (1u << log_n)) return;
  const uint32_t r = log_n ? (__brev(i) >> (32 - log_n)) : 0u;
  st28(out + r, ld28(in + i));
}

template <class F, bool DIF, bool LOCAL_TW, int THREADS>
__global__ void __launch_bounds__(THREADS)
k_ntt_pass(F* __restrict__ data, const F* __restrict__ tw, int log_n, int t0, int S, int Q,
           const F* __restrict__ post, uint32_t* __restrict__ canon_out) {
  data += (size_t)blockIdx.y << log_n;
  if (canon_out) canon_out += ((size_t)blockIdx.y << log_n) * 8;
  extern __shared__ __align__(16) unsigned char lds_raw[];
  F* tile = reinterpret_cast<F*>(lds_raw);
  const uint32_t tile_n = 1u << (S + Q);
  F* ctw = tile + tile_n;
  const uint32_t blk = blockIdx.x;
  const uint32_t mid_bits = (t0 > 0) ? (uint32_t)(t0 - Q) : 0u;
  const uint32_t mid = blk & ((1u << mid_bits) - 1u);
  const uint32_t hi = blk >> mid_bits;
  const uint32_t qeff = (t0 > 0) ? (uint32_t)Q : 0u;
  auto gindex = [&](uint32_t L) -> uint32_t {
    if (t0 == 0) return blk * tile_n + L;
    const uint32_t e = L >> Q, c = L & ((1u << Q) - 1u);
    return (hi << (t0 + S)) | (e << t0) | (mid << Q) | c;
  };
  auto twist = [&](uint32_t L) -> F {
    const uint32_t e = L >> Q, c = L & ((1u << Q) - 1u);
    const uint32_t col = (mid << Q) | c;
    const uint32_t ex = (col * (__brev(e) >> (32 - S))) << (log_n - t0 - S);
    const uint32_t halfn = 1u << (log_n - 1);
    F f = ld28(tw + (ex & (halfn - 1u)));
    return (ex & halfn) ? f.neg() : f;
  };
  if (LOCAL_TW)
    for (uint32_t k = threadIdx.x; k < (1u << (S - 1)); k += THREADS) ctw[k] = ld28(tw + ((size_t)k << (log_n - S)));
  for (uint32_t L = threadIdx.x; L < tile_n; L += THREADS) {
    F v = ld28(data + gindex(L));
    if (LOCAL_TW && !DIF && t0 > 0) v = v * twist(L);
    tile[L] = v;
  }
  __syncthreads();

  const uint32_t half = tile_n >> 1;
  for (int s = 0; s < S; s++) {
    const int u = DIF ? (S - 1 - s) : s;
    const int t = t0 + u;
    const uint32_t dist_log = (uint32_t)u + qeff;
    const uint32_t dist = 1u << dist_log;
    for (uint32_t b = threadIdx.x; b < half; b += THREADS) {
      const uint32_t lo = b & (dist - 1u);
      const uint32_t L0 = ((b >> dist_log) << (dist_log + 1)) | lo;
      const uint32_t L1 = L0 | dist;
      F w;
      if (LOCAL_TW) {
        w = ctw[(lo >> qeff) << (S - 1 - u)];
      } else {
        const uint32_t j = gindex(L0) & ((1u << t) - 1u);
        w = ld28(tw + ((size_t)j << (log_n - 1 - t)));
      }
      const F x = tile[L0];
      if (DIF) {
        const F y = tile[L1];
        tile[L0] = x + y;
        tile[L1] = x.sub_lazy(y) * w;
      } else {
        const F y = tile[L1] * w;
        tile[L0] = x + y;
        tile[L1] = x - y;
      }
    }
    __syncthreads();
  }

  for (uint32_t L = threadIdx.x; L < tile_n; L += THREADS) {
    const uint32_t g = gindex(L);
    F v = tile[L];
    if (LOCAL_TW && DIF && t0 > 0) v = v * twist(L);
    if (post) v = v * ld28(post + g);
    if (canon_out) {
      uint32_t w[8];
      v.to_canonical(w);
      st_words8(canon_out + (size_t)g * 8, w);
    } else {
      st28(data + g, v);
    }
  }
}

#ifdef ZKMI_EXPERIMENTS
#include "ntt_exp.hpp"
#endif

template <class F>
__global__ void __launch_bounds__(256)
k_mul_table(F* __restrict__ a, const F* __restrict__ b, uint32_t n) {
  const uint32_t i = blockIdx.x * blockDim.x + threadIdx.x;
  if (i < n) st28(a + i, ld28(a + i) * ld28(b + i));
}

template <class F>
__global__ void __launch_bounds__(256)
k_scale(F* __restrict__ a, F s, uint32_t n) {
  const uint32_t i = blockIdx.x * blockDim.x + threadIdx.x;
  if (i < n) st28(a + i, ld28(a + i) * s);
}

template <class F>
__global__ void __launch_bounds__(256)
k_power_table(F* __restrict__ out, F base, F first, uint32_t n) {
  const uint32_t i0 = (blockIdx.x * blockDim.x + threadIdx.x) * 16u;
  if (i0 >= n) return;
  F v = first, sq = base;
  for (uint32_t e = i0; e; e >>= 1) {
    if (e & 1u) v = v * sq;
    sq = sq * sq;
  }
  for (uint32_t k = 0; k < 16u && i0 + k < n; k++) {
    st28(out + i0 + k, v);
    v = v * base;
  }
}

template <class F>
__global__ void __launch_bounds__(256)
k_from_canonical(const uint32_t* __restrict__ in, F* __restrict__ out, uint32_t n) {
  const uint32_t i = blockIdx.x * blockDim.x + threadIdx.x;
  if (i >= n) return;
  uint32_t w[8];
  ld_words8(in + (size_t)i * 8, w);
  st28(out + i, F::from_canonical(w));
}
template <class F>
__global__ void __launch_bounds__(256)
k_to_canonical(const F* __restrict__ in, uint32_t* __restrict__ out, uint32_t n) {
  const uint32_t i = blockIdx.x * blockDim.x + threadIdx.x;
  if (i >= n) return;
  uint32_t w[8];
  ld28(in + i).to_canonical(w);
  st_words8(out + (size_t)i * 8, w);
}

}

Fr fr_root_of_unity(int log_n) {
  static const uint32_t ROOT_2_32[8] = {0x439f0d2bu, 0x3829971fu, 0x8c2280b9u, 0xb6368350u,
                                        0x22c813b4u, 0xd09b6819u, 0xdfe81f20u, 0x16a2a19eu};
  Fr w;
  for (int i = 0; i < 8; i++) w.l[i] = ROOT_2_32[i];
  w = w.to_mont();
  for (int i = 32; i > log_n; i--) w = w.sqr();
  return w;
}

NttField<Fr28>::Host NttField<Fr28>::root_max() { return fr_root_of_unity(32); }
NttField<BnFr28>::Host NttField<BnFr28>::root_max() {
  static const uint32_t ROOT_2_28[8] = {0x60c37c9cu, 0xd34f1ed9u, 0xd39329c8u, 0x3215cf6du,
                                        0x3dd31f74u, 0x98865ea9u, 0x166d18b7u, 0x03ddb9f5u};
  BnFr w;
  for (int i = 0; i < 8; i++) w.l[i] = ROOT_2_28[i];
  return w.to_mont();
}

template <class H>
static H host_from_u64(uint64_t v) {
  H a = H::zero();
  a.l[0] = (uint32_t)v;
  a.l[1] = (uint32_t)(v >> 32);
  return a.to_mont();
}
template <class F, class H>
static F to28(const H& a) {
  H c = a.from_mont();
  return F::from_canonical(c.l);
}

template <class F>
NttDomainT<F>::~NttDomainT() {
  F* ptrs[] = {tw_fwd, tw_inv, coset_fwd, coset_inv_n, rev_coset_n, rev_coset_inv_n, n_inv, scratch};
  for (F* p : ptrs)
    if (p) (void)hipFree(p);
}

template <class F>
hipError_t NttDomainT<F>::init(int log_n_, hipStream_t stream) {
  using H = typename NttField<F>::Host;
  if (log_n_ > NttField<F>::TWO_ADICITY) return hipErrorInvalidValue;
  log_n = log_n_;
  const uint32_t n = 1u << log_n;
  const uint32_t half = n > 1 ? n / 2 : 1;
  hipError_t e;
  F** alloc_n[] = {&coset_fwd, &coset_inv_n, &rev_coset_n, &rev_coset_inv_n, &scratch};
  if ((e = hipMalloc(&tw_fwd, sizeof(F) * half)) != hipSuccess) return e;
  if ((e = hipMalloc(&tw_inv, sizeof(F) * half)) != hipSuccess) return e;
  if ((e = hipMalloc(&n_inv, sizeof(F))) != hipSuccess) return e;
  for (F** p : alloc_n)
    if ((e = hipMalloc(p, sizeof(F) * n)) != hipSuccess) return e;
  H w = NttField<F>::root_max();
  for (int i = NttField<F>::TWO_ADICITY; i > log_n; i--) w = w.sqr();
  const H g = host_from_u64<H>(7);
  const H ninv = host_from_u64<H>(n).inv();
  const F one28 = F::one(), ninv28 = to28<F, H>(ninv);
  n_inv_host = ninv28;
  const int T = 256;
  auto blocks = [&](uint32_t cnt) { return (cnt + 16 * T - 1) / (16 * T); };
  hipLaunchKernelGGL(k_power_table<F>, dim3(blocks(half)), dim3(T), 0, stream, tw_fwd, to28<F, H>(w), one28, half);
  hipLaunchKernelGGL(k_power_table<F>, dim3(blocks(half)), dim3(T), 0, stream, tw_inv, to28<F, H>(w.inv()), one28, half);
  hipLaunchKernelGGL(k_power_table<F>, dim3(blocks(n)), dim3(T), 0, stream, coset_fwd, to28<F, H>(g), one28, n);
  hipLaunchKernelGGL(k_power_table<F>, dim3(blocks(n)), dim3(T), 0, stream, coset_inv_n, to28<F, H>(g.inv()), ninv28, n);
  hipLaunchKernelGGL(k_power_table<F>, dim3(blocks(n)), dim3(T), 0, stream, scratch, to28<F, H>(g), ninv28, n);
  hipLaunchKernelGGL(k_bitrev_copy<F>, dim3((n + T - 1) / T), dim3(T), 0, stream, scratch, rev_coset_n, log_n);
  hipLaunchKernelGGL(k_bitrev_copy<F>, dim3((n + T - 1) / T), dim3(T), 0, stream, coset_inv_n, rev_coset_inv_n, log_n);
  if ((e = hipMemcpyAsync(n_inv, &ninv28, sizeof(F), hipMemcpyHostToDevice, stream)) != hipSuccess) return e;
  if ((e = hipStreamSynchronize(stream)) != hipSuccess) return e;
  return hipGetLastError();
}

static int ntt_rb_mode() { return ZK_TUNE("ZKMI_NTT_RB", 6); }

#ifdef ZKMI_EXPERIMENTS
template <class F, bool DIF, bool LTW, int LOGE, int LOGR = 0, bool ONEW = false>
static void launch_rb(dim3 grid, uint32_t tile_n, int S, hipStream_t stream, F* buf, const F* tw, int log_n, int t0, int Q,
                      const F* post, uint32_t* canon_out) {
  const size_t words = (size_t)F::NL * (tile_n + (tile_n >> 5)) +
                       (LTW ? (size_t)F::NL * ((1u << (S - 1)) + ((1u << (S - 1)) >> 5) + 1u) : 0u);
  hipLaunchKernelGGL((k_ntt_pass_rb<F, DIF, LTW, LOGE, LOGR, ONEW>), grid, dim3(tile_n >> (LOGE + LOGR)), words * sizeof(uint32_t), stream,
                     buf, tw, log_n, t0, S, Q, post, canon_out);
}
#endif

template <class F, bool DIF>
static hipError_t run_passes(F* buf, const F* tw, int log_n, const F* post, uint32_t* canon_out,
                             hipStream_t stream, uint32_t batch = 1) {
  const uint32_t n = 1u << log_n;
  int mode = ntt_rb_mode();
  if (mode == 5 && log_n < 9) mode = 3;
  const int rb = (mode == 1 || mode == 2 || mode == 4 || mode == 5) ? mode : 0;
  const int tile_log = mode == 5 ? 9 : mode == 4 ? 10 : 11;
  struct Pass {
    int t0, S, Q;
  } passes[4];
  int np = 0;
  const int max_s = mode == 5 ? 9 : 10;
  const int want_np = (log_n + max_s - 1) / max_s;
  for (int t0 = 0; t0 < log_n;) {
    int S = log_n - t0;
    if (S > max_s) S = max_s;
    if (mode == 5) {
      const int left = want_np - np;
      S = (log_n - t0 + left - 1) / left;
    }
    int Q;
    if (rb) {
      Q = tile_log - S;
      const int room = (t0 > 0) ? t0 : (log_n - S);
      if (Q > room) Q = room;
    } else {
      Q = (t0 > 0) ? 1 : ((log_n > S) ? 1 : 0);
      if ((mode == 3 || mode == 6) && t0 > 0 && S < 10 && log_n - 11 >= 9) Q = (11 - S < t0) ? 11 - S : t0;
      if (mode == 6 && S + Q == 11) Q -= 1;
    }
    passes[np++] = {t0, S, Q};
    t0 += S;
  }
  const bool local3 = ZK_TUNE("ZKMI_NTT_LOCAL3", 0) == 1;
  const bool local_tw = np <= 2 || mode == 5 || local3;
  for (int k = 0; k < np; k++) {
    const Pass& p = DIF ? passes[np - 1 - k] : passes[k];
    const bool last = (k == np - 1);
    const uint32_t tile_n = 1u << (p.S + p.Q);
    const uint32_t nblk = n / tile_n;
    const F* pp = last ? post : nullptr;
    uint32_t* co = last ? canon_out : nullptr;
    const dim3 grid(nblk, batch);
#ifdef ZKMI_EXPERIMENTS
    if (rb == 5) {
      launch_rb<F, DIF, true, 2, 1, true>(grid, tile_n, p.S, stream, buf, tw, log_n, p.t0, p.Q, pp, co);
      continue;
    }
    if (rb == 4 && tile_n == 1024) {
      if (local_tw) launch_rb<F, DIF, true, 2, 2>(grid, tile_n, p.S, stream, buf, tw, log_n, p.t0, p.Q, pp, co);
      else launch_rb<F, DIF, false, 2, 2>(grid, tile_n, p.S, stream, buf, tw, log_n, p.t0, p.Q, pp, co);
      continue;
    }
    if (rb && rb != 4 && rb != 5 && tile_n >= 512) {
      if (rb == 2) {
        if (local_tw) launch_rb<F, DIF, true, 2>(grid, tile_n, p.S, stream, buf, tw, log_n, p.t0, p.Q, pp, co);
        else launch_rb<F, DIF, false, 2>(grid, tile_n, p.S, stream, buf, tw, log_n, p.t0, p.Q, pp, co);
      } else {
        if (local_tw) launch_rb<F, DIF, true, 3>(grid, tile_n, p.S, stream, buf, tw, log_n, p.t0, p.Q, pp, co);
        else launch_rb<F, DIF, false, 3>(grid, tile_n, p.S, stream, buf, tw, log_n, p.t0, p.Q, pp, co);
      }
      continue;
    }
#endif
    const size_t lds = ((size_t)tile_n + (local_tw ? (1u << (p.S - 1)) : 0u)) * sizeof(F);
    if (tile_n == 1024 && mode == 6) {
      if (local_tw)
        hipLaunchKernelGGL((k_ntt_pass<F, DIF, true, 512>), grid, dim3(512), lds, stream, buf, tw, log_n, p.t0, p.S, p.Q, pp, co);
      else
        hipLaunchKernelGGL((k_ntt_pass<F, DIF, false, 512>), grid, dim3(512), lds, stream, buf, tw, log_n, p.t0, p.S, p.Q, pp, co);
    } else if (tile_n >= 1024) {
      if (local_tw)
        hipLaunchKernelGGL((k_ntt_pass<F, DIF, true, 1024>), grid, dim3(1024), lds, stream, buf, tw, log_n, p.t0, p.S,
                           p.Q, pp, co);
      else
        hipLaunchKernelGGL((k_ntt_pass<F, DIF, false, 1024>), grid, dim3(1024), lds, stream, buf, tw, log_n, p.t0,
                           p.S, p.Q, pp, co);
    } else if (local_tw) {
      hipLaunchKernelGGL((k_ntt_pass<F, DIF, true, 64>), grid, dim3(64), lds, stream, buf, tw, log_n, p.t0, p.S, p.Q,
                         pp, co);
    } else {
      hipLaunchKernelGGL((k_ntt_pass<F, DIF, false, 64>), grid, dim3(64), lds, stream, buf, tw, log_n, p.t0, p.S, p.Q,
                         pp, co);
    }
  }
  return hipGetLastError();
}

template <class F>
hipError_t NttDomainT<F>::inverse_to_rev(F* d, const F* post_table, uint32_t* canon_out, hipStream_t st, uint32_t batch) {
  if (log_n == 0) {
    if (batch != 1) return hipErrorInvalidValue;
    if (post_table) hipLaunchKernelGGL(k_mul_table<F>, dim3(1), dim3(256), 0, st, d, post_table, 1u);
    if (canon_out) hipLaunchKernelGGL(k_to_canonical<F>, dim3(1), dim3(256), 0, st, d, canon_out, 1u);
    return hipGetLastError();
  }
  return run_passes<F, true>(d, tw_inv, log_n, post_table, canon_out, st, batch);
}

template <class F>
hipError_t NttDomainT<F>::forward_from_rev(F* d, hipStream_t st, uint32_t batch) {
  if (log_n == 0) return hipSuccess;
  return run_passes<F, false>(d, tw_fwd, log_n, nullptr, nullptr, st, batch);
}

template <class F>
hipError_t NttDomainT<F>::transform(F* d_data, bool inverse, bool coset, hipStream_t stream) {
  const uint32_t n = 1u << log_n;
  const int T = 256;
  if (coset && !inverse)
    hipLaunchKernelGGL(k_mul_table<F>, dim3((n + T - 1) / T), dim3(T), 0, stream, d_data, coset_fwd, n);
  if (log_n > 0) {
    hipLaunchKernelGGL(k_bitrev_copy<F>, dim3((n + T - 1) / T), dim3(T), 0, stream, d_data, scratch, log_n);
    hipError_t e = run_passes<F, false>(scratch, inverse ? tw_inv : tw_fwd, log_n, nullptr, nullptr, stream);
    if (e != hipSuccess) return e;
    if ((e = hipMemcpyAsync(d_data, scratch, sizeof(F) * n, hipMemcpyDeviceToDevice, stream)) != hipSuccess) return e;
  }
  if (inverse) {
    if (coset) {
      hipLaunchKernelGGL(k_mul_table<F>, dim3((n + T - 1) / T), dim3(T), 0, stream, d_data, coset_inv_n, n);
    } else {
      hipLaunchKernelGGL(k_scale<F>, dim3((n + T - 1) / T), dim3(T), 0, stream, d_data, n_inv_host, n);
    }
  }
  return hipGetLastError();
}

template <class F>
hipError_t ntt_from_canonical(const uint32_t* d_in, F* d_out, uint32_t n, hipStream_t s) {
  if (!n) return hipSuccess;
  hipLaunchKernelGGL(k_from_canonical<F>, dim3((n + 63) / 64), dim3(64), 0, s, d_in, d_out, n);
  return hipGetLastError();
}
template <class F>
hipError_t ntt_to_canonical(const F* d_in, uint32_t* d_out, uint32_t n, hipStream_t s) {
  if (!n) return hipSuccess;
  hipLaunchKernelGGL(k_to_canonical<F>, dim3((n + 255) / 256), dim3(256), 0, s, d_in, d_out, n);
  return hipGetLastError();
}
template <class F>
hipError_t ntt_mul_table(F* d, const F* table, uint32_t n, hipStream_t s) {
  if (!n) return hipSuccess;
  hipLaunchKernelGGL(k_mul_table<F>, dim3((n + 255) / 256), dim3(256), 0, s, d, table, n);
  return hipGetLastError();
}

#ifdef ZKMI_EXPERIMENTS
template <class F>
static hipError_t rb_enable_big_lds() {
  const void* fns[] = {reinterpret_cast<const void*>(k_ntt_pass_rb<F, true, true, 3>),  reinterpret_cast<const void*>(k_ntt_pass_rb<F, false, true, 3>),
                       reinterpret_cast<const void*>(k_ntt_pass_rb<F, true, false, 3>), reinterpret_cast<const void*>(k_ntt_pass_rb<F, false, false, 3>),
                       reinterpret_cast<const void*>(k_ntt_pass_rb<F, true, true, 2>),  reinterpret_cast<const void*>(k_ntt_pass_rb<F, false, true, 2>),
                       reinterpret_cast<const void*>(k_ntt_pass_rb<F, true, false, 2>), reinterpret_cast<const void*>(k_ntt_pass_rb<F, false, false, 2>),
                       reinterpret_cast<const void*>((k_ntt_pass_rb<F, true, true, 2, 2>)),  reinterpret_cast<const void*>((k_ntt_pass_rb<F, false, true, 2, 2>)),
                       reinterpret_cast<const void*>((k_ntt_pass_rb<F, true, false, 2, 2>)), reinterpret_cast<const void*>((k_ntt_pass_rb<F, false, false, 2, 2>)),
                       reinterpret_cast<const void*>((k_ntt_pass_rb<F, true, true, 2, 1, true>)), reinterpret_cast<const void*>((k_ntt_pass_rb<F, false, true, 2, 1, true>))};
  for (const void* f : fns) {
    const hipError_t e = hipFuncSetAttribute(f, hipFuncAttributeMaxDynamicSharedMemorySize, 160 * 1024);
    if (e != hipSuccess) return e;
  }
  return hipSuccess;
}
#endif

hipError_t ntt_enable_big_lds() {
  const void* fns[] = {reinterpret_cast<const void*>(k_ntt_pass<Fr28, true, true, 1024>),
                       reinterpret_cast<const void*>(k_ntt_pass<Fr28, false, true, 1024>),
                       reinterpret_cast<const void*>(k_ntt_pass<Fr28, true, false, 1024>),
                       reinterpret_cast<const void*>(k_ntt_pass<Fr28, false, false, 1024>),
                       reinterpret_cast<const void*>(k_ntt_pass<BnFr28, true, true, 1024>),
                       reinterpret_cast<const void*>(k_ntt_pass<BnFr28, false, true, 1024>),
                       reinterpret_cast<const void*>(k_ntt_pass<BnFr28, true, false, 1024>),
                       reinterpret_cast<const void*>(k_ntt_pass<BnFr28, false, false, 1024>),
                       reinterpret_cast<const void*>(k_ntt_pass<Fr28, true, true, 512>),
                       reinterpret_cast<const void*>(k_ntt_pass<Fr28, false, true, 512>),
                       reinterpret_cast<const void*>(k_ntt_pass<Fr28, true, false, 512>),
                       reinterpret_cast<const void*>(k_ntt_pass<Fr28, false, false, 512>),
                       reinterpret_cast<const void*>(k_ntt_pass<BnFr28, true, true, 512>),
                       reinterpret_cast<const void*>(k_ntt_pass<BnFr28, false, true, 512>),
                       reinterpret_cast<const void*>(k_ntt_pass<BnFr28, true, false, 512>),
                       reinterpret_cast<const void*>(k_ntt_pass<BnFr28, false, false, 512>)};
  for (const void* f : fns) {
    hipError_t e = hipFuncSetAttribute(f, hipFuncAttributeMaxDynamicSharedMemorySize, 160 * 1024);
    if (e != hipSuccess) return e;
  }
#ifdef ZKMI_EXPERIMENTS
  hipError_t e = rb_enable_big_lds<Fr28>();
  if (e == hipSuccess) e = rb_enable_big_lds<BnFr28>();
  return e;
#else
  return hipSuccess;
#endif
}

template struct NttDomainT<Fr28>;
template struct NttDomainT<BnFr28>;
template hipError_t ntt_from_canonical<Fr28>(const uint32_t*, Fr28*, uint32_t, hipStream_t);
template hipError_t ntt_to_canonical<Fr28>(const Fr28*, uint32_t*, uint32_t, hipStream_t);
template hipError_t ntt_mul_table<Fr28>(Fr28*, const Fr28*, uint32_t, hipStream_t);
template hipError_t ntt_from_canonical<BnFr28>(const uint32_t*, BnFr28*, uint32_t, hipStream_t);
template hipError_t ntt_to_canonical<BnFr28>(const BnFr28*, uint32_t*, uint32_t, hipStream_t);
template hipError_t ntt_mul_table<BnFr28>(BnFr28*, const BnFr28*, uint32_t, hipStream_t);

}
```

### zk-apps_amd/csrc/ntt.hpp

```cpp
#pragma once
#include "field28.hpp"

namespace zkmi {

template <class F>
__device__ __forceinline__ F ld28(const F* p) {
  static_assert(F::NL == 10, "10-limb scalar fields");
  F r;
  const uint2* q = reinterpret_cast<const uint2*>(p);
#pragma unroll
  for (int i = 0; i < 5; i++) {
    const uint2 v = q[i];
    r.l[2 * i] = (int32_t)v.x;
    r.l[2 * i + 1] = (int32_t)v.y;
  }
  return r;
}
template <class F>
__device__ __forceinline__ void st28(F* p, const F& v) {
  uint2* q = reinterpret_cast<uint2*>(p);
#pragma unroll
  for (int i = 0; i < 5; i++) q[i] = make_uint2((uint32_t)v.l[2 * i], (uint32_t)v.l[2 * i + 1]);
}

template <class F> struct NttField;
template <> struct NttField<Fr28> {
  using Host = Fr;
  static constexpr int TWO_ADICITY = 32;
  static Host root_max();
};
template <> struct NttField<BnFr28> {
  using Host = BnFr;
  static constexpr int TWO_ADICITY = 28;
  static Host root_max();
};

template <class F>
struct NttDomainT {
  int log_n = 0;
  F* tw_fwd = nullptr;
  F* tw_inv = nullptr;
  F* coset_fwd = nullptr;
  F* coset_inv_n = nullptr;
  F* rev_coset_n = nullptr;
  F* rev_coset_inv_n = nullptr;
  F* n_inv = nullptr;
  F* scratch = nullptr;
  F n_inv_host;
  ~NttDomainT();
  hipError_t init(int log_n, hipStream_t stream);
  hipError_t transform(F* d_data, bool inverse, bool coset, hipStream_t stream);
  hipError_t inverse_to_rev(F* d, const F* post_table, uint32_t* canon_out, hipStream_t st, uint32_t batch = 1);
  hipError_t forward_from_rev(F* d, hipStream_t st, uint32_t batch = 1);
};

using NttDomain = NttDomainT<Fr28>;
using NttDomainBn = NttDomainT<BnFr28>;

Fr fr_root_of_unity(int log_n);
template <class F> hipError_t ntt_from_canonical(const uint32_t* d_in, F* d_out, uint32_t n, hipStream_t s);
template <class F> hipError_t ntt_to_canonical(const F* d_in, uint32_t* d_out, uint32_t n, hipStream_t s);
template <class F> hipError_t ntt_mul_table(F* d, const F* table, uint32_t n, hipStream_t s);
hipError_t ntt_enable_big_lds();

}
```

### zk-apps_amd/csrc/ntt_exp.hpp

```cpp
template <int... Is, class Fn>
__device__ __forceinline__ void static_for_impl(std::integer_sequence<int, Is...>, Fn&& f) {
  (f(std::integral_constant<int, Is>{}), ...);
}
template <int N, class Fn>
__device__ __forceinline__ void static_for(Fn&& f) {
  static_for_impl(std::make_integer_sequence<int, N>{}, f);
}

template <class F>
struct RbLds {
  uint32_t* w;
  uint32_t pitch;
  __device__ __forceinline__ static uint32_t pad(uint32_t L) { return L + (L >> 5); }
  __device__ __forceinline__ F ld(uint32_t L) const {
    F r;
    const uint32_t o = pad(L);
#pragma unroll
    for (int i = 0; i < F::NL; i++) r.l[i] = (int32_t)w[i * pitch + o];
    return r;
  }
  __device__ __forceinline__ void st(uint32_t L, const F& v) const {
    const uint32_t o = pad(L);
#pragma unroll
    for (int i = 0; i < F::NL; i++) w[i * pitch + o] = (uint32_t)v.l[i];
  }
};

template <class F, bool DIF, bool LOCAL_TW, int LOGE, int LOGR = 0, bool ONEW = false>
__global__ void __launch_bounds__((LOGR || ONEW) ? 64 : (2048 >> LOGE), ONEW ? 3 : 1)
k_ntt_pass_rb(F* __restrict__ data, const F* __restrict__ tw, int log_n, int t0, int S, int Q,
              const F* __restrict__ post, uint32_t* __restrict__ canon_out) {
  constexpr int E = 1 << LOGE;
  constexpr int REP = 1 << LOGR;
  data += (size_t)blockIdx.y << log_n;
  if (canon_out) canon_out += ((size_t)blockIdx.y << log_n) * 8;
  extern __shared__ __align__(16) unsigned char lds_raw[];
  const uint32_t tile_n = 1u << (S + Q);
  const uint32_t nthr = tile_n >> (LOGE + LOGR);
  const uint32_t nunit = tile_n >> LOGE;
  RbLds<F> tile{reinterpret_cast<uint32_t*>(lds_raw), tile_n + (tile_n >> 5)};
  RbLds<F> ctw{tile.w + (size_t)F::NL * tile.pitch, (1u << (S - 1)) + ((1u << (S - 1)) >> 5) + 1u};
  const uint32_t blk = blockIdx.x, tid = threadIdx.x;
  const uint32_t mid_bits = (t0 > 0) ? (uint32_t)(t0 - Q) : 0u;
  const uint32_t mid = blk & ((1u << mid_bits) - 1u);
  const uint32_t hi = blk >> mid_bits;
  const uint32_t qeff = (t0 > 0) ? (uint32_t)Q : 0u;
  auto gindex = [&](uint32_t L) -> uint32_t {
    if (t0 == 0) return blk * tile_n + L;
    const uint32_t e = L >> Q, c = L & ((1u << Q) - 1u);
    return (hi << (t0 + S)) | (e << t0) | (mid << Q) | c;
  };
  auto twist = [&](uint32_t L) -> F {
    const uint32_t e = L >> Q, c = L & ((1u << Q) - 1u);
    const uint32_t col = (mid << Q) | c;
    const uint32_t ex = (col * (__brev(e) >> (32 - S))) << (log_n - t0 - S);
    const uint32_t halfn = 1u << (log_n - 1);
    F f = ld28(tw + (ex & (halfn - 1u)));
    return (ex & halfn) ? f.neg() : f;
  };
  if (LOCAL_TW)
    for (uint32_t k = tid; k < (1u << (S - 1)); k += nthr) ctw.st(k, ld28(tw + ((size_t)k << (log_n - S))));
#pragma unroll
  for (int m = 0; m < E * REP; m++) {
    const uint32_t L = tid + (uint32_t)m * nthr;
    F v = ld28(data + gindex(L));
    if (LOCAL_TW && !DIF && t0 > 0) v = v * twist(L);
    tile.st(L, v);
  }
  __syncthreads();

  auto round = [&](auto kc, int u0) __attribute__((always_inline)) {
    constexpr int K = decltype(kc)::value;
    const uint32_t sh = (uint32_t)u0 + qeff;
    for (uint32_t unit = tid; unit < nunit; unit += nthr) {
    F x[E];
    uint32_t Lm[E];
    static_for<E>([&](auto mc) __attribute__((always_inline)) {
      constexpr int m = decltype(mc)::value;
      constexpr uint32_t j = (uint32_t)m & ((1u << K) - 1u), g = (uint32_t)m >> K;
      const uint32_t G = (unit << (LOGE - K)) | g;
      Lm[m] = ((G >> sh) << (sh + K)) | (G & ((1u << sh) - 1u)) | (j << sh);
      x[m] = tile.ld(Lm[m]);
    });
    static_for<K>([&](auto ic) __attribute__((always_inline)) {
      constexpr int i = DIF ? (K - 1 - decltype(ic)::value) : decltype(ic)::value;
      const int u = u0 + i;
      const uint32_t dist_log = (uint32_t)u + qeff;
      static_for<E>([&](auto m0c) __attribute__((always_inline)) {
        constexpr int m0 = decltype(m0c)::value;
        if constexpr ((m0 & (1 << i)) == 0) {
          constexpr int m1 = m0 | (1 << i);
          F w;
          if (LOCAL_TW) {
            const uint32_t lo = Lm[m0] & ((1u << dist_log) - 1u);
            w = ctw.ld((lo >> qeff) << (S - 1 - u));
          } else {
            const int t = t0 + u;
            const uint32_t jj = gindex(Lm[m0]) & ((1u << t) - 1u);
            w = ld28(tw + ((size_t)jj << (log_n - 1 - t)));
          }
          if (DIF) {
            const F a = x[m0], b = x[m1];
            x[m0] = a + b;
            x[m1] = a.sub_lazy(b) * w;
          } else {
            const F y = x[m1] * w;
            const F a = x[m0];
            x[m0] = a + y;
            x[m1] = a - y;
          }
        }
      });
    });
    static_for<E>([&](auto mc) __attribute__((always_inline)) {
      constexpr int m = decltype(mc)::value;
      tile.st(Lm[m], x[m]);
    });
    }
    __syncthreads();
  };
  {
    int done = 0;
    while (done < S) {
      int k = S - done;
      if (k > LOGE) k = LOGE;
      const int u0 = DIF ? (S - done - k) : done;
      if (LOGE >= 3 && k == 3) round(std::integral_constant<int, (LOGE >= 3 ? 3 : 1)>{}, u0);
      else if (LOGE >= 2 && k == 2) round(std::integral_constant<int, (LOGE >= 2 ? 2 : 1)>{}, u0);
      else round(std::integral_constant<int, 1>{}, u0);
      done += k;
    }
  }

#pragma unroll
  for (int m = 0; m < E * REP; m++) {
    const uint32_t L = tid + (uint32_t)m * nthr;
    const uint32_t g = gindex(L);
    F v = tile.ld(L);
    if (LOCAL_TW && DIF && t0 > 0) v = v * twist(L);
    if (post) v = v * ld28(post + g);
    if (canon_out) {
      uint32_t w[8];
      v.to_canonical(w);
      st_words8(canon_out + (size_t)g * 8, w);
    } else {
      st28(data + g, v);
    }
  }
}
```

Baseline: 58.06 proofs/s.

## Skip C forward NTT via linearity and add second-level segment reduction in MSM

The quotient step now drops the forward coset NTT of C. It computes A*B on the coset, scales C's coefficients by n, and subtracts them inside the last inverse NTT pass. A new post-table rev_quot_n handles the zinv and coset factors. This removes one of the seven Fr NTTs per proof. Separately, the MSM reduction gains a second-level segment-sum kernel that folds 16 segments at once, so the tree-sum kernels process fewer entries. This changes the job count and the host-side window reconstruction, and depends on the new table being initialised correctly.

Result: faster. 60.09 proofs/s, median of 6 (+3.5%).

```diff
diff --git a/zk-apps_amd/csrc/groth16.hip b/zk-apps_amd/csrc/groth16.hip
--- a/zk-apps_amd/csrc/groth16.hip
+++ b/zk-apps_amd/csrc/groth16.hip
@@ -132,10 +132,11 @@
 }
 
 __global__ void __launch_bounds__(256)
-k_quotient(Fr28* __restrict__ a, const Fr28* __restrict__ b, const Fr28* __restrict__ c, Fr28 zinv, uint32_t n) {
+k_quotient(Fr28* __restrict__ a, const Fr28* __restrict__ b, Fr28* __restrict__ c, Fr28 n_field, uint32_t n) {
   const uint32_t i = blockIdx.x * blockDim.x + threadIdx.x;
   if (i >= n) return;
-  st28(a + i, (ld28(a + i) * ld28(b + i) - ld28(c + i)) * zinv);
+  st28(a + i, ld28(a + i) * ld28(b + i));
+  st28(c + i, ld28(c + i) * n_field);
 }
 
 struct ZPtrSet {
@@ -826,19 +827,15 @@
   const bool batch_abc = ZK_TUNE("ZKMI_WITNESS_BATCH", 1) != 0;
   if (batch_abc) {
     ZK_HIP(ctx, dom->inverse_to_rev(pk->d_a, dom->rev_coset_n, nullptr, st, 3 * G));
-    ZK_HIP(ctx, dom->forward_from_rev(pk->d_a, st, 3 * G));
+    ZK_HIP(ctx, dom->forward_from_rev(pk->d_a, st, 2 * G));
   } else {
     for (int m = 0; m < 3; m++) {
       ZK_HIP(ctx, dom->inverse_to_rev(pk->d_a + (size_t)m * N * G, dom->rev_coset_n, nullptr, st, G));
-      ZK_HIP(ctx, dom->forward_from_rev(pk->d_a + (size_t)m * N * G, st, G));
-    }
-  }
-  Fr gn = fr_from_u64(7);
-  for (uint32_t i = 0; i < pk->log_n; i++) gn = gn.sqr();
-  const Fr zinv = (gn - Fr::one()).inv().from_mont();
-  const Fr28 zinv28 = Fr28::from_canonical(zinv.l);
-  hipLaunchKernelGGL(k_quotient, dim3((G * N + 63) / 64), dim3(64), 0, st, pk->d_a, d_b, d_c, zinv28, G * N);
-  ZK_HIP(ctx, dom->inverse_to_rev(pk->d_a, dom->rev_coset_inv_n, pk->d_h[par], st, G));
+      if (m < 2) ZK_HIP(ctx, dom->forward_from_rev(pk->d_a + (size_t)m * N * G, st, G));
+    }
+  }
+  hipLaunchKernelGGL(k_quotient, dim3((G * N + 63) / 64), dim3(64), 0, st, pk->d_a, d_b, d_c, dom->n_host, G * N);
+  ZK_HIP(ctx, dom->inverse_to_rev(pk->d_a, dom->rev_quot_n, pk->d_h[par], st, G, d_c));
   if (t) t->end(PH_NTT, st);
   if (st != ctx->stream) ZK_HIP(ctx, hipEventRecord(ctx->ev_h[par], st));
   ZK_HIP(ctx, hipGetLastError());
diff --git a/zk-apps_amd/csrc/msm.hpp b/zk-apps_amd/csrc/msm.hpp
--- a/zk-apps_amd/csrc/msm.hpp
+++ b/zk-apps_amd/csrc/msm.hpp
@@ -50,6 +50,7 @@
   uint32_t heavy_thr = 256;
   int heavy_shift = 0;
   int seg_log = 4;
+  int seg2_log = 0;
   int vec_parts = 1;
   int top_spread_log = 0;
   int win_first = 0, nwin_total = 0;
@@ -112,6 +113,7 @@
   XYZZ<F>* buckets = nullptr;
   XYZZ<F>* segsum = nullptr;
   XYZZ<F>* segw = nullptr;
+  XYZZ<F>* seg2 = nullptr;
   uint64_t seg_cap = 0;
   XYZZ<F>* heavy_partial = nullptr;
   uint32_t* heavy_ticket = nullptr;
diff --git a/zk-apps_amd/csrc/msm_impl.hpp b/zk-apps_amd/csrc/msm_impl.hpp
--- a/zk-apps_amd/csrc/msm_impl.hpp
+++ b/zk-apps_amd/csrc/msm_impl.hpp
@@ -10,6 +10,8 @@
 namespace zkmi {
 
 static inline uint64_t msm_max_segments(uint64_t buckets) { return (buckets / 16 > (1u << 16) ? buckets / 16 : (1u << 16)) + 1; }
+constexpr int MSM_SEG2_LOG = 4;
+constexpr uint32_t MSM_SEG2_MIN_SEGS = 256;
 constexpr int MSM_TREE_T = 128;
 constexpr uint32_t MSM_STAGE_PTS = 16384;
 constexpr uint32_t MSM_STAGE_PTS_1 = 4096;
@@ -988,18 +990,74 @@
 }
 
 template <class F>
+__global__ void __launch_bounds__(256)
+k_segreduce2(const XYZZ<F>* __restrict__ segsum, XYZZ<F>* __restrict__ segsum2, XYZZ<F>* __restrict__ segt2, uint32_t total_segs2) {
+  const uint32_t u = blockIdx.x * blockDim.x + threadIdx.x;
+  if (u >= total_segs2) return;
+  XYZZ<F> run = XYZZ<F>::infinity();
+  XYZZ<F> acc = XYZZ<F>::infinity();
+  for (int k = (1 << MSM_SEG2_LOG) - 1; k >= 0; k--) {
+    XYZZ<F> v = load_vec(segsum + ((size_t)u << MSM_SEG2_LOG) + k);
+    run.add(v);
+    if (k) acc.add(run);
+  }
+  store_vec(segsum2 + u, run);
+  store_vec(segt2 + u, acc);
+}
+template <int UNUSED = 0>
+__global__ void __launch_bounds__(256, 2)
+k_segreduce2_g2_split(const XYZZ<Fq2_28>* __restrict__ segsum, XYZZ<Fq2_28>* __restrict__ segsum2, XYZZ<Fq2_28>* __restrict__ segt2,
+                      uint32_t total_segs2) {
+  const uint32_t gt = blockIdx.x * blockDim.x + threadIdx.x;
+  const uint32_t u = gt >> 1, comp = gt & 1u;
+  if (u >= total_segs2) return;
+  XYZZ<Fq2P> run = XYZZ<Fq2P>::infinity();
+  XYZZ<Fq2P> acc = XYZZ<Fq2P>::infinity();
+  for (int k = (1 << MSM_SEG2_LOG) - 1; k >= 0; k--) {
+    XYZZ<Fq2P> v = ld_xyzz_split(segsum + ((size_t)u << MSM_SEG2_LOG) + k, comp);
+    run.add(v);
+    if (k) acc.add(run);
+  }
+  st_xyzz_split(segsum2 + u, run, comp);
+  st_xyzz_split(segt2 + u, acc, comp);
+}
+
+template <class P>
+struct TreeLevel2 {
+  const P* segsum2;
+  const P* segt2;
+  uint32_t segs2;
+  int t_job;
+};
+template <class P>
+__device__ __forceinline__ const P* tree_job_list(int job, int w, const P* segsum, const P* segw, uint32_t segs_per_win, int plain_job,
+                                                  const TreeLevel2<P>& l2, uint32_t* len, bool* whole) {
+  *whole = job == 0 || job == plain_job || job == l2.t_job;
+  if (job == 0) {
+    *len = segs_per_win;
+    return segw + (size_t)w * segs_per_win;
+  }
+  if (l2.t_job < 0) {
+    *len = *whole ? segs_per_win : segs_per_win / 2;
+    return segsum + (size_t)w * segs_per_win;
+  }
+  *len = *whole ? l2.segs2 : l2.segs2 / 2;
+  return (job == l2.t_job ? l2.segt2 : l2.segsum2) + (size_t)w * l2.segs2;
+}
+
+template <class F>
 __global__ void __launch_bounds__(MSM_TREE_T)
 k_treesum(const XYZZ<F>* __restrict__ segsum, const XYZZ<F>* __restrict__ segw, uint32_t segs_per_win,
           XYZZ<typename HostFieldOf<F>::type>* __restrict__ partial, int plain_job, XYZZ<F>* __restrict__ stage,
-          XYZZ<typename HostFieldOf<F>::type>* __restrict__ partial_host) {
+          XYZZ<typename HostFieldOf<F>::type>* __restrict__ partial_host, TreeLevel2<XYZZ<F>> l2) {
   extern __shared__ __align__(16) unsigned char lds_raw[];
   XYZZ<F>* sh = reinterpret_cast<XYZZ<F>*>(lds_raw);
   const int job = blockIdx.x;
   const int w = blockIdx.y;
   const uint32_t nchunk = gridDim.z, z = blockIdx.z;
-  const XYZZ<F>* src = (job == 0 ? segw : segsum) + (size_t)w * segs_per_win;
-  const bool whole = job == 0 || job == plain_job;
-  const uint32_t len = whole ? segs_per_win : segs_per_win / 2;
+  uint32_t len;
+  bool whole;
+  const XYZZ<F>* src = tree_job_list(job, w, segsum, segw, segs_per_win, plain_job, l2, &len, &whole);
   const uint32_t per = (len + nchunk - 1) / nchunk;
   const uint32_t lo = z * per, hi = lo + per < len ? lo + per : len;
   XYZZ<F> acc = XYZZ<F>::infinity();
@@ -1086,16 +1144,17 @@
 template <int UNUSED = 0>
 __global__ void __launch_bounds__(2 * MSM_TREE_T, 2)
 k_treesum_g2_split(const XYZZ<Fq2_28>* __restrict__ segsum, const XYZZ<Fq2_28>* __restrict__ segw, uint32_t segs_per_win,
-                   XYZZ<Fq2>* __restrict__ partial, int plain_job, XYZZ<Fq2_28>* __restrict__ stage, XYZZ<Fq2>* __restrict__ partial_host) {
+                   XYZZ<Fq2>* __restrict__ partial, int plain_job, XYZZ<Fq2_28>* __restrict__ stage, XYZZ<Fq2>* __restrict__ partial_host,
+                   TreeLevel2<XYZZ<Fq2_28>> l2) {
   extern __shared__ __align__(16) unsigned char lds_raw[];
   XYZZ<Fq2_28>* sh = reinterpret_cast<XYZZ<Fq2_28>*>(lds_raw);
   const int job = blockIdx.x;
   const int w = blockIdx.y;
   const uint32_t nchunk = gridDim.z, z = blockIdx.z;
   const uint32_t pair = threadIdx.x >> 1, comp = threadIdx.x & 1u, npair = blockDim.x >> 1;
-  const XYZZ<Fq2_28>* src = (job == 0 ? segw : segsum) + (size_t)w * segs_per_win;
-  const bool whole = job == 0 || job == plain_job;
-  const uint32_t len = whole ? segs_per_win : segs_per_win / 2;
+  uint32_t len;
+  bool whole;
+  const XYZZ<Fq2_28>* src = tree_job_list(job, w, segsum, segw, segs_per_win, plain_job, l2, &len, &whole);
   const uint32_t per = (len + nchunk - 1) / nchunk;
   const uint32_t lo = z * per, hi = lo + per < len ? lo + per : len;
   const uint32_t b = whole ? 0u : (uint32_t)(job - 1), lowmask = (1u << b) - 1u;
@@ -1270,6 +1329,8 @@
   if (buckets) (void)hipFree(buckets);
   if (segsum) (void)hipFree(segsum);
   if (segw) (void)hipFree(segw);
+  if (seg2) (void)hipFree(seg2);
+  seg2 = nullptr;
   if (partial) (void)hipFree(partial);
   if (tree_stage) (void)hipFree(tree_stage);
   tree_stage = nullptr;
@@ -1351,6 +1412,7 @@
   seg_cap = msm_max_segments(need);
   if ((e = hipMalloc(&segsum, sizeof(XYZZ<F>) * seg_cap * nslots)) != hipSuccess) return e;
   if ((e = hipMalloc(&segw, sizeof(XYZZ<F>) * seg_cap * nslots)) != hipSuccess) return e;
+  if ((e = hipMalloc(&seg2, sizeof(XYZZ<F>) * 2 * (seg_cap >> MSM_SEG2_LOG) * nslots)) != hipSuccess) return e;
   if ((e = hipMalloc(&partial, sizeof(XYZZ<HF>) * SLOTS * SLOT_PTS)) != hipSuccess) return e;
   if ((e = hipMalloc(&tree_stage, sizeof(XYZZ<F>) * MSM_STAGE_PTS * nslots)) != hipSuccess) return e;
   if ((e = hipMalloc(&heavy_partial, sizeof(XYZZ<F>) * ((size_t)MSM_HPOOL + MSM_HNC_POOL) * nslots)) != hipSuccess) return e;
@@ -1374,6 +1436,10 @@
   int seg_bits = 0;
   while ((1u << seg_bits) < segs_per_win) seg_bits++;
   return seg_bits;
+}
+static inline int msm_njobs(const MsmPlan& pl) {
+  if (pl.seg2_log) return 3 + msm_seg_bits(pl) - pl.seg2_log;
+  return 1 + msm_seg_bits(pl) + (pl.shared ? 1 : 0);
 }
 
 template <class F>
@@ -1490,8 +1556,10 @@
       hipLaunchKernelGGL(k_mask_sorted<0>, dim3(1024), dim3(256), 0, st, sorts[m]->sorted, sorts[m]->cap_entries,
                          0x80000000u | ((1u << mask_bits) - 1u));
 #endif
+  const bool level2 = pl.shared && !(quad_mask & 3) && (pl.nb >> pl.seg_log) >= MSM_SEG2_MIN_SEGS;
   for (int m = 0; m < nm; m++) {
     slot_plan[slots[m]] = sorts[m]->plan;
+    slot_plan[slots[m]].seg2_log = level2 ? MSM_SEG2_LOG : 0;
     const hipStream_t st_reduce = st_reduces[m];
     const bool on_reduce = heavy_on == 2 && st_reduce != st;
     const bool side = !on_reduce && heavy_on != 0 && st_heavy && st_heavy != st;
@@ -1641,8 +1709,10 @@
   const uint32_t segs_per_win = pl.nb >> pl.seg_log;
   const uint32_t tot_segs = pl.nwin * segs_per_win;
   const int seg = 1 << pl.seg_log;
-  const int plain_job = pl.shared ? 1 + msm_seg_bits(pl) : -1;
-  const int njobs = 1 + msm_seg_bits(pl) + (pl.shared ? 1 : 0);
+  const uint32_t segs2 = segs_per_win >> MSM_SEG2_LOG, tot_segs2 = tot_segs >> MSM_SEG2_LOG;
+  const int njobs = msm_njobs(slot_plan[slots[0]]);
+  const int plain_job = pl.shared ? njobs - 1 : -1;
+  const int t_job = level2 ? njobs - 2 : -1;
   constexpr bool is_g2 = std::is_same<F, Fq2_28>::value;
   const uint32_t per_block = is_g2 ? MSM_TREE_T : 2 * MSM_TREE_T;
   uint32_t nchunk = 1;
@@ -1717,6 +1787,16 @@
       else
         hipLaunchKernelGGL(k_segreduce<F>, dim3((tot_segs + T - 1) / T), dim3(T), 0, st_reduce, bk, ssum, sw, tot_segs, seg, bk2, bk3);
     }
+    TreeLevel2<XYZZ<F>> l2 = {nullptr, nullptr, 0u, -1};
+    if (level2) {
+      XYZZ<F>* const s2 = seg2 + (size_t)slot * 2 * (seg_cap >> MSM_SEG2_LOG);
+      XYZZ<F>* const t2 = s2 + (seg_cap >> MSM_SEG2_LOG);
+      if constexpr (is_g2)
+        hipLaunchKernelGGL(k_segreduce2_g2_split<0>, dim3((2 * tot_segs2 + T - 1) / T), dim3(T), 0, st_reduce, ssum, s2, t2, tot_segs2);
+      else
+        hipLaunchKernelGGL(k_segreduce2<F>, dim3((tot_segs2 + T - 1) / T), dim3(T), 0, st_reduce, ssum, s2, t2, tot_segs2);
+      l2 = {s2, t2, segs2, t_job};
+    }
     XYZZ<HF>* dp = partial + (size_t)slot * SLOT_PTS;
     XYZZ<HF>* const hp_out = h_partial + (size_t)slot * SLOT_PTS;
     XYZZ<F>* const stg = tree_stage + (size_t)slot * MSM_STAGE_PTS;
@@ -1729,7 +1809,7 @@
     } else if constexpr (is_g2) {
       if (nchunk > 1) {
         hipLaunchKernelGGL(k_treesum_g2_split<0>, dim3(njobs, pl.nwin, nchunk), dim3(MSM_TREE_T), sizeof(XYZZ<F>) * MSM_TREE_T / 2, st_reduce,
-                           ssum, sw, segs_per_win, dp, plain_job, stg, hp_out);
+                           ssum, sw, segs_per_win, dp, plain_job, stg, hp_out, l2);
         uint32_t tf = 64;
         while (tf < 2 * nchunk) tf <<= 1;
         hipLaunchKernelGGL(k_treesum_final_g2_split<0>, dim3(njobs, pl.nwin), dim3(tf), sizeof(XYZZ<F>) * tf / 2, st_reduce, stg, nchunk, dp, hp_out);
@@ -1737,15 +1817,15 @@
 #ifdef ZKMI_EXPERIMENTS
         if (ZK_TUNE("ZKMI_G2_TREE_SPLIT", 1) == 0)
           hipLaunchKernelGGL(k_treesum<F>, dim3(njobs, pl.nwin, 1), dim3(MSM_TREE_T), sizeof(XYZZ<F>) * MSM_TREE_T, st_reduce,
-                             ssum, sw, segs_per_win, dp, plain_job, stg, hp_out);
+                             ssum, sw, segs_per_win, dp, plain_job, stg, hp_out, l2);
         else
 #endif
           hipLaunchKernelGGL(k_treesum_g2_split<0>, dim3(njobs, pl.nwin, 1), dim3(2 * MSM_TREE_T), sizeof(XYZZ<F>) * MSM_TREE_T, st_reduce,
-                             ssum, sw, segs_per_win, dp, plain_job, stg, hp_out);
+                             ssum, sw, segs_per_win, dp, plain_job, stg, hp_out, l2);
       }
     } else {
       hipLaunchKernelGGL(k_treesum<F>, dim3(njobs, pl.nwin, nchunk), dim3(MSM_TREE_T), sizeof(XYZZ<F>) * MSM_TREE_T, st_reduce,
-                         ssum, sw, segs_per_win, dp, plain_job, stg, hp_out);
+                         ssum, sw, segs_per_win, dp, plain_job, stg, hp_out, l2);
       if (nchunk > 1) {
         uint32_t tf = 64;
         while (tf < nchunk) tf <<= 1;
@@ -1767,17 +1847,21 @@
 }
 
 template <class F>
-int MsmEngine<F>::partials_per_msm(const MsmPlan& pl) { return pl.nwin * (1 + msm_seg_bits(pl) + (pl.shared ? 1 : 0)); }
+int MsmEngine<F>::partials_per_msm(const MsmPlan& pl) { return pl.nwin * msm_njobs(pl); }
 template <class F>
 void MsmEngine<F>::windows_from_partials(const MsmPlan& pl, const XYZZ<HF>* h, XYZZ<HF>* out_windows, bool parallel) {
-  const int seg_bits = msm_seg_bits(pl);
-  const int njobs = 1 + seg_bits + (pl.shared ? 1 : 0);
+  const int seg_bits = msm_seg_bits(pl) - pl.seg2_log;
+  const int njobs = msm_njobs(pl);
   const std::function<void(uint32_t)> one = [&](uint32_t w) {
     XYZZ<HF> u = XYZZ<HF>::infinity();
     const int bits = (pl.win_first + (int)w == pl.total_windows() - 1 && pl.top_spread_log > 0) ? seg_bits - pl.top_spread_log : seg_bits;
     for (int j = bits - 1; j >= 0; j--) {
       u.dbl_inplace();
       u.add(h[(size_t)w * njobs + 1 + j]);
+    }
+    if (pl.seg2_log) {
+      for (int i = 0; i < pl.seg2_log; i++) u.dbl_inplace();
+      u.add(h[(size_t)w * njobs + njobs - 2]);
     }
     for (int i = 0; i < pl.seg_log; i++) u.dbl_inplace();
     u.add(h[(size_t)w * njobs]);
@@ -1810,7 +1894,7 @@
   std::vector<XYZZ<HF>> win(pl.nwin);
   hipError_t e = finish_host_windows(win.data(), slot);
   if (e != hipSuccess) return e;
-  const int njobs = 2 + msm_seg_bits(pl);
+  const int njobs = msm_njobs(pl);
   const XYZZ<HF>* h = h_partial + (size_t)slot * SLOT_PTS;
   for (int v = 0; v * pl.vec_parts < pl.nwin; v++)
     out[v] = msm_combine_partitions<HF>(win.data() + (size_t)v * pl.vec_parts, h + (size_t)v * pl.vec_parts * njobs, pl.vec_parts,
@@ -1826,7 +1910,7 @@
 XYZZ<typename MsmEngine<F>::HF> MsmEngine<F>::host_result_vec(int slot, int v) const {
   const MsmPlan& pl = slot_plan[slot];
   const int vp = pl.vec_parts > 1 ? pl.vec_parts : 1;
-  const int njobs = 1 + msm_seg_bits(pl) + (pl.shared ? 1 : 0);
+  const int njobs = msm_njobs(pl);
   const XYZZ<HF>* h = h_partial + (size_t)slot * SLOT_PTS + (size_t)v * vp * njobs;
   MsmPlan mine = pl;
   mine.nwin = vp;
@@ -1856,7 +1940,7 @@
     *out = msm_combine_windows(win.data(), pl.nwin, pl.c);
     return hipSuccess;
   }
-  *out = msm_combine_partitions<HF>(win.data(), h_partial + (size_t)slot * SLOT_PTS, pl.nwin, 2 + msm_seg_bits(pl), pl.nb);
+  *out = msm_combine_partitions<HF>(win.data(), h_partial + (size_t)slot * SLOT_PTS, pl.nwin, msm_njobs(pl), pl.nb);
   return hipSuccess;
 }
 
diff --git a/zk-apps_amd/csrc/ntt.hip b/zk-apps_amd/csrc/ntt.hip
--- a/zk-apps_amd/csrc/ntt.hip
+++ b/zk-apps_amd/csrc/ntt.hip
@@ -31,8 +31,9 @@
 template <class F, bool DIF, bool LOCAL_TW, int THREADS>
 __global__ void __launch_bounds__(THREADS)
 k_ntt_pass(F* __restrict__ data, const F* __restrict__ tw, int log_n, int t0, int S, int Q,
-           const F* __restrict__ post, uint32_t* __restrict__ canon_out) {
+           const F* __restrict__ post, const F* __restrict__ sub, uint32_t* __restrict__ canon_out) {
   data += (size_t)blockIdx.y << log_n;
+  if (sub) sub += (size_t)blockIdx.y << log_n;
   if (canon_out) canon_out += ((size_t)blockIdx.y << log_n) * 8;
   extern __shared__ __align__(16) unsigned char lds_raw[];
   F* tile = reinterpret_cast<F*>(lds_raw);
@@ -100,6 +101,7 @@
     const uint32_t g = gindex(L);
     F v = tile[L];
     if (LOCAL_TW && DIF && t0 > 0) v = v * twist(L);
+    if (sub) v = v - ld28(sub + g);
     if (post) v = v * ld28(post + g);
     if (canon_out) {
       uint32_t w[8];
@@ -120,6 +122,13 @@
 k_mul_table(F* __restrict__ a, const F* __restrict__ b, uint32_t n) {
   const uint32_t i = blockIdx.x * blockDim.x + threadIdx.x;
   if (i < n) st28(a + i, ld28(a + i) * ld28(b + i));
+}
+
+template <class F>
+__global__ void __launch_bounds__(256)
+k_sub(F* __restrict__ a, const F* __restrict__ b, uint32_t n) {
+  const uint32_t i = blockIdx.x * blockDim.x + threadIdx.x;
+  if (i < n) st28(a + i, ld28(a + i) - ld28(b + i));
 }
 
 template <class F>
@@ -200,7 +209,7 @@
 
 template <class F>
 NttDomainT<F>::~NttDomainT() {
-  F* ptrs[] = {tw_fwd, tw_inv, coset_fwd, coset_inv_n, rev_coset_n, rev_coset_inv_n, n_inv, scratch};
+  F* ptrs[] = {tw_fwd, tw_inv, coset_fwd, coset_inv_n, rev_coset_n, rev_quot_n, n_inv, scratch};
   for (F* p : ptrs)
     if (p) (void)hipFree(p);
 }
@@ -213,7 +222,7 @@
   const uint32_t n = 1u << log_n;
   const uint32_t half = n > 1 ? n / 2 : 1;
   hipError_t e;
-  F** alloc_n[] = {&coset_fwd, &coset_inv_n, &rev_coset_n, &rev_coset_inv_n, &scratch};
+  F** alloc_n[] = {&coset_fwd, &coset_inv_n, &rev_coset_n, &rev_quot_n, &scratch};
   if ((e = hipMalloc(&tw_fwd, sizeof(F) * half)) != hipSuccess) return e;
   if ((e = hipMalloc(&tw_inv, sizeof(F) * half)) != hipSuccess) return e;
   if ((e = hipMalloc(&n_inv, sizeof(F))) != hipSuccess) return e;
@@ -233,7 +242,12 @@
   hipLaunchKernelGGL(k_power_table<F>, dim3(blocks(n)), dim3(T), 0, stream, coset_inv_n, to28<F, H>(g.inv()), ninv28, n);
   hipLaunchKernelGGL(k_power_table<F>, dim3(blocks(n)), dim3(T), 0, stream, scratch, to28<F, H>(g), ninv28, n);
   hipLaunchKernelGGL(k_bitrev_copy<F>, dim3((n + T - 1) / T), dim3(T), 0, stream, scratch, rev_coset_n, log_n);
-  hipLaunchKernelGGL(k_bitrev_copy<F>, dim3((n + T - 1) / T), dim3(T), 0, stream, coset_inv_n, rev_coset_inv_n, log_n);
+  H gn = g;
+  for (int i = 0; i < log_n; i++) gn = gn.sqr();
+  const H zinv = (gn - H::one()).inv();
+  n_host = to28<F, H>(host_from_u64<H>(n));
+  hipLaunchKernelGGL(k_power_table<F>, dim3(blocks(n)), dim3(T), 0, stream, scratch, to28<F, H>(g.inv()), to28<F, H>(ninv * zinv), n);
+  hipLaunchKernelGGL(k_bitrev_copy<F>, dim3((n + T - 1) / T), dim3(T), 0, stream, scratch, rev_quot_n, log_n);
   if ((e = hipMemcpyAsync(n_inv, &ninv28, sizeof(F), hipMemcpyHostToDevice, stream)) != hipSuccess) return e;
   if ((e = hipStreamSynchronize(stream)) != hipSuccess) return e;
   return hipGetLastError();
@@ -244,16 +258,16 @@
 #ifdef ZKMI_EXPERIMENTS
 template <class F, bool DIF, bool LTW, int LOGE, int LOGR = 0, bool ONEW = false>
 static void launch_rb(dim3 grid, uint32_t tile_n, int S, hipStream_t stream, F* buf, const F* tw, int log_n, int t0, int Q,
-                      const F* post, uint32_t* canon_out) {
+                      const F* post, const F* sub, uint32_t* canon_out) {
   const size_t words = (size_t)F::NL * (tile_n + (tile_n >> 5)) +
                        (LTW ? (size_t)F::NL * ((1u << (S - 1)) + ((1u << (S - 1)) >> 5) + 1u) : 0u);
   hipLaunchKernelGGL((k_ntt_pass_rb<F, DIF, LTW, LOGE, LOGR, ONEW>), grid, dim3(tile_n >> (LOGE + LOGR)), words * sizeof(uint32_t), stream,
-                     buf, tw, log_n, t0, S, Q, post, canon_out);
+                     buf, tw, log_n, t0, S, Q, post, sub, canon_out);
 }
 #endif
 
 template <class F, bool DIF>
-static hipError_t run_passes(F* buf, const F* tw, int log_n, const F* post, uint32_t* canon_out,
+static hipError_t run_passes(F* buf, const F* tw, int log_n, const F* post, const F* sub, uint32_t* canon_out,
                              hipStream_t stream, uint32_t batch = 1) {
   const uint32_t n = 1u << log_n;
   int mode = ntt_rb_mode();
@@ -294,25 +308,26 @@
     const uint32_t tile_n = 1u << (p.S + p.Q);
     const uint32_t nblk = n / tile_n;
     const F* pp = last ? post : nullptr;
+    const F* sb = last ? sub : nullptr;
     uint32_t* co = last ? canon_out : nullptr;
     const dim3 grid(nblk, batch);
 #ifdef ZKMI_EXPERIMENTS
     if (rb == 5) {
-      launch_rb<F, DIF, true, 2, 1, true>(grid, tile_n, p.S, stream, buf, tw, log_n, p.t0, p.Q, pp, co);
+      launch_rb<F, DIF, true, 2, 1, true>(grid, tile_n, p.S, stream, buf, tw, log_n, p.t0, p.Q, pp, sb, co);
       continue;
     }
     if (rb == 4 && tile_n == 1024) {
-      if (local_tw) launch_rb<F, DIF, true, 2, 2>(grid, tile_n, p.S, stream, buf, tw, log_n, p.t0, p.Q, pp, co);
-      else launch_rb<F, DIF, false, 2, 2>(grid, tile_n, p.S, stream, buf, tw, log_n, p.t0, p.Q, pp, co);
+      if (local_tw) launch_rb<F, DIF, true, 2, 2>(grid, tile_n, p.S, stream, buf, tw, log_n, p.t0, p.Q, pp, sb, co);
+      else launch_rb<F, DIF, false, 2, 2>(grid, tile_n, p.S, stream, buf, tw, log_n, p.t0, p.Q, pp, sb, co);
       continue;
     }
     if (rb && rb != 4 && rb != 5 && tile_n >= 512) {
       if (rb == 2) {
-        if (local_tw) launch_rb<F, DIF, true, 2>(grid, tile_n, p.S, stream, buf, tw, log_n, p.t0, p.Q, pp, co);
-        else launch_rb<F, DIF, false, 2>(grid, tile_n, p.S, stream, buf, tw, log_n, p.t0, p.Q, pp, co);
+        if (local_tw) launch_rb<F, DIF, true, 2>(grid, tile_n, p.S, stream, buf, tw, log_n, p.t0, p.Q, pp, sb, co);
+        else launch_rb<F, DIF, false, 2>(grid, tile_n, p.S, stream, buf, tw, log_n, p.t0, p.Q, pp, sb, co);
       } else {
-        if (local_tw) launch_rb<F, DIF, true, 3>(grid, tile_n, p.S, stream, buf, tw, log_n, p.t0, p.Q, pp, co);
-        else launch_rb<F, DIF, false, 3>(grid, tile_n, p.S, stream, buf, tw, log_n, p.t0, p.Q, pp, co);
+        if (local_tw) launch_rb<F, DIF, true, 3>(grid, tile_n, p.S, stream, buf, tw, log_n, p.t0, p.Q, pp, sb, co);
+        else launch_rb<F, DIF, false, 3>(grid, tile_n, p.S, stream, buf, tw, log_n, p.t0, p.Q, pp, sb, co);
       }
       continue;
     }
@@ -320,42 +335,45 @@
     const size_t lds = ((size_t)tile_n + (local_tw ? (1u << (p.S - 1)) : 0u)) * sizeof(F);
     if (tile_n == 1024 && mode == 6) {
       if (local_tw)
-        hipLaunchKernelGGL((k_ntt_pass<F, DIF, true, 512>), grid, dim3(512), lds, stream, buf, tw, log_n, p.t0, p.S, p.Q, pp, co);
+        hipLaunchKernelGGL((k_ntt_pass<F, DIF, true, 512>), grid, dim3(512), lds, stream, buf, tw, log_n, p.t0, p.S, p.Q, pp, sb, co);
       else
-        hipLaunchKernelGGL((k_ntt_pass<F, DIF, false, 512>), grid, dim3(512), lds, stream, buf, tw, log_n, p.t0, p.S, p.Q, pp, co);
+        hipLaunchKernelGGL((k_ntt_pass<F, DIF, false, 512>), grid, dim3(512), lds, stream, buf, tw, log_n, p.t0, p.S, p.Q, pp, sb, co);
     } else if (tile_n >= 1024) {
       if (local_tw)
         hipLaunchKernelGGL((k_ntt_pass<F, DIF, true, 1024>), grid, dim3(1024), lds, stream, buf, tw, log_n, p.t0, p.S,
-                           p.Q, pp, co);
+                           p.Q, pp, sb, co);
       else
         hipLaunchKernelGGL((k_ntt_pass<F, DIF, false, 1024>), grid, dim3(1024), lds, stream, buf, tw, log_n, p.t0,
-                           p.S, p.Q, pp, co);
+                           p.S, p.Q, pp, sb, co);
     } else if (local_tw) {
       hipLaunchKernelGGL((k_ntt_pass<F, DIF, true, 64>), grid, dim3(64), lds, stream, buf, tw, log_n, p.t0, p.S, p.Q,
-                         pp, co);
+                         pp, sb, co);
     } else {
       hipLaunchKernelGGL((k_ntt_pass<F, DIF, false, 64>), grid, dim3(64), lds, stream, buf, tw, log_n, p.t0, p.S, p.Q,
-                         pp, co);
-    }
-  }
-  return hipGetLastError();
-}
-
-template <class F>
-hipError_t NttDomainT<F>::inverse_to_rev(F* d, const F* post_table, uint32_t* canon_out, hipStream_t st, uint32_t batch) {
+                         pp, sb, co);
+    }
+  }
+  return hipGetLastError();
+}
+
+template <class F>
+hipError_t NttDomainT<F>::inverse_to_rev(F* d, const F* post_table, uint32_t* canon_out, hipStream_t st, uint32_t batch,
+                                         const F* sub) {
+  if (sub && !post_table) return hipErrorInvalidValue;
   if (log_n == 0) {
     if (batch != 1) return hipErrorInvalidValue;
+    if (sub) hipLaunchKernelGGL(k_sub<F>, dim3(1), dim3(256), 0, st, d, sub, 1u);
     if (post_table) hipLaunchKernelGGL(k_mul_table<F>, dim3(1), dim3(256), 0, st, d, post_table, 1u);
     if (canon_out) hipLaunchKernelGGL(k_to_canonical<F>, dim3(1), dim3(256), 0, st, d, canon_out, 1u);
     return hipGetLastError();
   }
-  return run_passes<F, true>(d, tw_inv, log_n, post_table, canon_out, st, batch);
+  return run_passes<F, true>(d, tw_inv, log_n, post_table, sub, canon_out, st, batch);
 }
 
 template <class F>
 hipError_t NttDomainT<F>::forward_from_rev(F* d, hipStream_t st, uint32_t batch) {
   if (log_n == 0) return hipSuccess;
-  return run_passes<F, false>(d, tw_fwd, log_n, nullptr, nullptr, st, batch);
+  return run_passes<F, false>(d, tw_fwd, log_n, nullptr, nullptr, nullptr, st, batch);
 }
 
 template <class F>
@@ -366,7 +384,7 @@
     hipLaunchKernelGGL(k_mul_table<F>, dim3((n + T - 1) / T), dim3(T), 0, stream, d_data, coset_fwd, n);
   if (log_n > 0) {
     hipLaunchKernelGGL(k_bitrev_copy<F>, dim3((n + T - 1) / T), dim3(T), 0, stream, d_data, scratch, log_n);
-    hipError_t e = run_passes<F, false>(scratch, inverse ? tw_inv : tw_fwd, log_n, nullptr, nullptr, stream);
+    hipError_t e = run_passes<F, false>(scratch, inverse ? tw_inv : tw_fwd, log_n, nullptr, nullptr, nullptr, stream);
     if (e != hipSuccess) return e;
     if ((e = hipMemcpyAsync(d_data, scratch, sizeof(F) * n, hipMemcpyDeviceToDevice, stream)) != hipSuccess) return e;
   }
diff --git a/zk-apps_amd/csrc/ntt.hpp b/zk-apps_amd/csrc/ntt.hpp
--- a/zk-apps_amd/csrc/ntt.hpp
+++ b/zk-apps_amd/csrc/ntt.hpp
@@ -43,14 +43,16 @@
   F* coset_fwd = nullptr;
   F* coset_inv_n = nullptr;
   F* rev_coset_n = nullptr;
-  F* rev_coset_inv_n = nullptr;
+  F* rev_quot_n = nullptr;
   F* n_inv = nullptr;
   F* scratch = nullptr;
   F n_inv_host;
+  F n_host;
   ~NttDomainT();
   hipError_t init(int log_n, hipStream_t stream);
   hipError_t transform(F* d_data, bool inverse, bool coset, hipStream_t stream);
-  hipError_t inverse_to_rev(F* d, const F* post_table, uint32_t* canon_out, hipStream_t st, uint32_t batch = 1);
+  hipError_t inverse_to_rev(F* d, const F* post_table, uint32_t* canon_out, hipStream_t st, uint32_t batch = 1,
+                            const F* sub = nullptr);
   hipError_t forward_from_rev(F* d, hipStream_t st, uint32_t batch = 1);
 };
 
diff --git a/zk-apps_amd/csrc/ntt_exp.hpp b/zk-apps_amd/csrc/ntt_exp.hpp
--- a/zk-apps_amd/csrc/ntt_exp.hpp
+++ b/zk-apps_amd/csrc/ntt_exp.hpp
@@ -29,10 +29,11 @@
 template <class F, bool DIF, bool LOCAL_TW, int LOGE, int LOGR = 0, bool ONEW = false>
 __global__ void __launch_bounds__((LOGR || ONEW) ? 64 : (2048 >> LOGE), ONEW ? 3 : 1)
 k_ntt_pass_rb(F* __restrict__ data, const F* __restrict__ tw, int log_n, int t0, int S, int Q,
-              const F* __restrict__ post, uint32_t* __restrict__ canon_out) {
+              const F* __restrict__ post, const F* __restrict__ sub, uint32_t* __restrict__ canon_out) {
   constexpr int E = 1 << LOGE;
   constexpr int REP = 1 << LOGR;
   data += (size_t)blockIdx.y << log_n;
+  if (sub) sub += (size_t)blockIdx.y << log_n;
   if (canon_out) canon_out += ((size_t)blockIdx.y << log_n) * 8;
   extern __shared__ __align__(16) unsigned char lds_raw[];
   const uint32_t tile_n = 1u << (S + Q);
@@ -138,6 +139,7 @@
     const uint32_t g = gindex(L);
     F v = tile.ld(L);
     if (LOCAL_TW && DIF && t0 > 0) v = v * twist(L);
+    if (sub) v = v - ld28(sub + g);
     if (post) v = v * ld28(post + g);
     if (canon_out) {
       uint32_t w[8];
```
